# yangjunjie0320/fft-isdf-scratch

Measured on AMD Instinct MI355X. Metric: ISDF build + get_jk k-points/s, diamond gth-dzvp 4x4x4, higher is better.
Workload: dtype f64 (complex128)

## Files before the change

fft-isdf-scratch_amd/csrc/api.hip:

```cpp
#include "../../include/fisdf.h"

#include <algorithm>
#include <cstdlib>
#include <cmath>
#include <cstring>
#include <functional>
#include <map>
#include <mutex>
#include <set>
#include <string>
#include <vector>

#include "common.h"
#include "linalg.h"

namespace fisdf {

static thread_local std::string g_last_error;
static thread_local fisdf_ctx* t_cur_ctx = nullptr;
static std::mutex g_live_mu;
static std::set<const fisdf_ctx*> g_live;
void set_ctx_error(fisdf_ctx* c, const std::string& msg);
void set_error(const std::string& msg) {
  g_last_error = msg;
// ... 56 lines not shown
  bool time_reversal = false;
  double omega = 0.0;
  hipStream_t aux[3] = {nullptr, nullptr, nullptr};
  hipEvent_t ev_fork = nullptr, ev_join[3] = {nullptr, nullptr, nullptr};
  unsigned aux_use[3] = {0, 0, 0}, aux_joined[3] = {0, 0, 0};
  hipEvent_t ev_ybuf[4] = {nullptr, nullptr, nullptr, nullptr};
  std::vector<hipEvent_t> ev_q;
  std::vector<hipEvent_t> ev_free;
  int pipe_mode = -1;
  int pipe_depth = 0;
  int last_fit_lanes = 0, last_fit_pipe = 0;
  struct FitRec {
    int v[12] = {0, 0, 0, 0, 0, 0, 0, 0, 0, 0, 0, 0};
  };
  std::vector<FitRec> fit_report;
  std::vector<hipEvent_t> ev_ready;
  std::vector<char> ready_marked;
  std::vector<const cplx*> y_piece;
  bool y_real_store = false;
  std::vector<char> y_real_slot;
  std::vector<long> y_slices;
  std::map<std::vector<long>, PlaneRef*> plane_cache;
  int* f_piv = nullptr;
  int* f_rank_dev = nullptr;
  std::vector<int> f_rank;
  hipStream_t side = nullptr;
  int factor_hi = 0, side_hi = -1;
  std::vector<hipStream_t> pad;
  void* pad_buf = nullptr;
  hipEvent_t ev_x4 = nullptr, ev_fac = nullptr, ev_chol = nullptr;
  hipEvent_t ev_fac_early = nullptr;
  int f_early = 0;
  bool f_fac_unjoined = false;
  bool f_pending = false;
  bool x4_marked = false;
  int* f_rank_pinned = nullptr;
  void* f_scratch = nullptr;
  size_t f_scratch_size = 0;
  int* stage_pinned = nullptr;
  int* sel_pinned = nullptr;
  size_t sel_cap = 0;
  size_t stage_cap = 0;
  hipEvent_t ev_stage = nullptr;
  unsigned long long* maximag = nullptr;
  unsigned long long* trmon = nullptr;
  unsigned long long* tr_pinned = nullptr;
  hipEvent_t ev_tr = nullptr;
  bool timing = false;
  struct Ev { int stage; hipEvent_t a, b; int span; };
  std::vector<Ev> events;
  unsigned long long* spans = nullptr;
  int span_used = 0;
  static constexpr int kSpanCap = 16384;
  std::string last_error;
  struct Build {
    bool valid = false;
    int nk = 0, nip = 0, nao = 0, ng0 = 0, nfit = 0, used_pivoted = 0, min_norm = 0;
    int time_reversal = 0;
    double tr_deviation = 0.0;
    int kmesh[3] = {0, 0, 0}, mesh[3] = {0, 0, 0};
    double a[9] = {0};
    std::vector<int> perm, fit_qs, partner, ranks;
    std::vector<double> wt;
    void *X = nullptr, *x4 = nullptr, *Wq = nullptr, *Ws = nullptr;
    int shard_rank = 0, shard_size = 1, row0 = 0, row1 = 0;
    void* W0 = nullptr;
    bool sharded = false;
    bool y_streamed = false;
    fisdf_comm comm{};
  } bld;
  hipStream_t comm_stream = nullptr;
  hipEvent_t ev_comm = nullptr;
  fisdf_alloc_fn alloc_fn = nullptr;
  fisdf_free_fn free_fn = nullptr;
  void* alloc_user = nullptr;
  std::map<int, std::pair<void*, size_t>> owned;
  std::vector<void*> lent;
  int* ys_dev = nullptr;
  int* ys_err_pinned = nullptr;
  hipEvent_t ev_yerr = nullptr;
  hipEvent_t ev_ysfork = nullptr;
  hipEvent_t ev_ys2[2] = {nullptr, nullptr};
  DevBuf ws_ypiv, ws_ystream;
  struct YStream {
    bool armed = false, enqueued = false;
    bool stale = false;
    int aux = 2;
    const cplx* x0 = nullptr;
    const cplx* f = nullptr;
    int ng0 = 0, nao = 0, nip = 0, rows = 128;
    long m = 0, fks = 0;
    int kmesh[3] = {0, 0, 0};
    std::vector<int> qs;
    cplx* yT = nullptr;
    unsigned long long rmask = 0;
  } ys;
};

namespace fisdf {
void set_ctx_error(fisdf_ctx* c, const std::string& msg) { c->last_error = msg; }
}

namespace {

static int devbuf_get(fisdf_ctx::DevBuf& w, size_t bytes, void** out) {
  bytes = std::max<size_t>(bytes, 256);
  if (bytes > w.n) {
    if (w.p) {
      FISDF_HIP(hipDeviceSynchronize());
      FISDF_HIP(hipFree(w.p));
    }
    w.p = nullptr;
    w.n = 0;
    FISDF_HIP(hipMalloc(&w.p, bytes));
    w.n = bytes;
  }
  *out = w.p;
  return 0;
}

int arena_get(fisdf_ctx* c, size_t bytes, void** out) {
  bytes = std::max<size_t>(bytes, 256);
  if (bytes > c->arena_size) {
    FISDF_HIP(hipStreamSynchronize(c->stream));
    if (c->arena) FISDF_HIP(hipFree(c->arena));
    c->arena = nullptr;
    c->arena_size = 0;
    size_t sz = bytes + bytes / 8;
    if (hipMalloc(&c->arena, sz) != hipSuccess) {
      (void)hipGetLastError();
      c->arena = nullptr;
      FISDF_HIP(hipMalloc(&c->arena, bytes));
      sz = bytes;
    }
    c->arena_size = sz;
  }
  *out = c->arena;
  return 0;
}

struct Carver {
  size_t off = 0;
  size_t take(size_t bytes) {
    size_t o = off;
    off += (bytes + 255) / 256 * 256;
    return o;
  }
};

int upload_bytes(fisdf_ctx* c, const void* h, size_t bytes, void* d) {
  if (bytes == 0) return 0;
  if (!c->ev_stage) FISDF_HIP(hipEventCreateWithFlags(&c->ev_stage, hipEventDisableTiming));
  FISDF_HIP(hipEventSynchronize(c->ev_stage));
  if (bytes > c->stage_cap) {
    if (c->stage_pinned) FISDF_HIP(hipHostFree(c->stage_pinned));
    c->stage_pinned = nullptr;
    c->stage_cap = 0;
    FISDF_HIP(hipHostMalloc((void**)&c->stage_pinned, bytes, hipHostMallocDefault));
    c->stage_cap = bytes;
  }
  std::memcpy(c->stage_pinned, h, bytes);
  FISDF_HIP(hipMemcpyAsync(d, c->stage_pinned, bytes, hipMemcpyHostToDevice, c->stream));
  FISDF_HIP(hipEventRecord(c->ev_stage, c->stream));
  return 0;
}

// ... 415 lines not shown
}


int pick_ksplit(int M, int N, int K) {
  long tiles = (long)((M + 63) / 64) * ((N + 63) / 64);
  int ks = 1;
  while (tiles * ks < 1024 && K / (ks * 2) >= 512) ks *= 2;
  return ks;
}

constexpr int kLaneWppMinQ = 12;
bool lane_wpp_wanted(int nq) {
  static const int lane_wpp_env = [] {
    const char* e = getenv("FISDF_LANE_WPP");
    return e ? atoi(e) : -1;
  }();
  return lane_wpp_env < 0 ? nq >= kLaneWppMinQ : lane_wpp_env != 0;
}

int wpp_ksplit(int nip) {
  const char* e = getenv("FISDF_WPP_KSPLIT");
  const int v = e ? atoi(e) : 4;
  return (nip >= 256 && v > 1) ? std::min(v, 16) : 1;
}

}

extern "C" {

int fisdf_abi_version(void) { return FISDF_ABI_VERSION; }

const char* fisdf_last_error(const fisdf_ctx* c) {
  return c ? c->last_error.c_str() : g_last_error.c_str();
}

int fisdf_create(int device, void* stream, fisdf_ctx** out) {
  t_cur_ctx = nullptr;
  FISDF_CHECK(out != nullptr, "out is null");
  int ndev = 0;
  FISDF_HIP(hipGetDeviceCount(&ndev));
  FISDF_CHECK(device >= 0 && device < ndev, "device id out of range (no GPU visible?)");
  FISDF_HIP(hipSetDevice(device));
  fisdf_ctx* c = new fisdf_ctx();
  c->device = device;
  c->stream = (hipStream_t)stream;
  c->own_stream = false;
  FISDF_HIP(hipMalloc(&c->maximag, 4 * sizeof(unsigned long long)));
  FISDF_HIP(hipMemsetAsync(c->maximag, 0, 4 * sizeof(unsigned long long), c->stream));
  {
    std::lock_guard<std::mutex> lk(g_live_mu);
    g_live.insert(c);
  }
  *out = c;
  return 0;
}

int fisdf_destroy(fisdf_ctx* c) {
  if (!c) return 0;
  {
    std::lock_guard<std::mutex> lk(g_live_mu);
    g_live.erase(c);
  }
  if (t_cur_ctx == c) t_cur_ctx = nullptr;
  FISDF_HIP(hipSetDevice(c->device));
  FISDF_HIP(hipStreamSynchronize(c->stream));
  c->lent.clear();
  for (auto& kv : c->owned)
    if (kv.second.first) (void)hipFree(kv.second.first);
  c->owned.clear();
  for (auto& e : c->events) { (void)hipEventDestroy(e.a); (void)hipEventDestroy(e.b); }
  for (auto& kv : c->phase_cache) (void)hipFree(kv.second);
  for (auto& kv : c->asym_cache) {
    (void)hipFree(kv.second.idx);
    if (kv.second.f) (void)hipFree(kv.second.f);
  }
  for (auto& kv : c->wt_cache) (void)hipFree(kv.second);
  if (c->f_pending) (void)hipEventSynchronize(c->ev_fac);
  free_factors(c);
  if (c->f_scratch) (void)hipFree(c->f_scratch);
  if (c->f_ring) (void)hipFree(c->f_ring);
  for (int l = 0; l < 3; ++l)
    if (c->aux[l]) (void)hipStreamSynchronize(c->aux[l]);
  if (c->ys_dev) (void)hipFree(c->ys_dev);
  if (c->ys_err_pinned) (void)hipHostFree(c->ys_err_pinned);
  if (c->ev_yerr) (void)hipEventDestroy(c->ev_yerr);
  if (c->ev_ysfork) (void)hipEventDestroy(c->ev_ysfork);
  for (hipEvent_t e : c->ev_ys2)
    if (e) (void)hipEventDestroy(e);
  for (auto* w : {&c->ws_main, &c->ws_side_a, &c->ws_side_b, &c->ws_x4, &c->ws_ypiv, &c->ws_ystream})
    if (w->p) (void)hipFree(w->p);
  for (hipStream_t p : c->pad) (void)hipStreamDestroy(p);
  if (c->pad_buf) (void)hipFree(c->pad_buf);
  if (c->side) {
    (void)hipStreamSynchronize(c->side);
    (void)hipStreamDestroy(c->side);
    (void)hipEventDestroy(c->ev_x4);
    (void)hipEventDestroy(c->ev_fac);
    (void)hipEventDestroy(c->ev_fac_early);
    (void)hipEventDestroy(c->ev_chol);
  }
  if (c->ev_fork) {
    (void)hipEventDestroy(c->ev_fork);
    for (int l = 0; l < 3; ++l) {
      if (c->aux[l]) {
        (void)hipStreamSynchronize(c->aux[l]);
        (void)hipStreamDestroy(c->aux[l]);
        c->aux[l] = nullptr;
      }
      (void)hipEventDestroy(c->ev_join[l]);
    }
    for (int l = 0; l < 4; ++l) (void)hipEventDestroy(c->ev_ybuf[l]);
  }
  for (hipEvent_t e : c->ev_q) (void)hipEventDestroy(e);
  for (hipEvent_t e : c->ev_free) (void)hipEventDestroy(e);
  for (hipEvent_t e : c->ev_ready) (void)hipEventDestroy(e);
  if (c->comm_stream) {
    (void)hipStreamSynchronize(c->comm_stream);
    (void)hipStreamDestroy(c->comm_stream);
    (void)hipEventDestroy(c->ev_comm);
  }
  for (auto& kv : c->plane_cache) (void)hipFree(kv.second);
  if (c->arena) (void)hipFree(c->arena);
  if (c->ev_stage) (void)hipEventSynchronize(c->ev_stage), (void)hipEventDestroy(c->ev_stage);
  if (c->stage_pinned) (void)hipHostFree(c->stage_pinned);
  if (c->sel_pinned) (void)hipHostFree(c->sel_pinned);
  if (c->maximag) (void)hipFree(c->maximag);
  if (c->ev_tr) (void)hipEventSynchronize(c->ev_tr), (void)hipEventDestroy(c->ev_tr);
  if (c->trmon) (void)hipFree(c->trmon);
  if (c->tr_pinned) (void)hipHostFree(c->tr_pinned);
  if (c->spans) (void)hipFree(c->spans);
  if (c->own_stream) (void)hipStreamDestroy(c->stream);
  delete c;
  return 0;
}

int fisdf_sync(fisdf_ctx* c) {
  FISDF_TRY(device_guard(c));
  FISDF_HIP(hipStreamSynchronize(c->stream));
  return 0;
}

int fisdf_malloc(fisdf_ctx* c, size_t bytes, void** p) {
  FISDF_TRY(device_guard(c));
  FISDF_HIP(hipMalloc(p, std::max<size_t>(bytes, 1)));
  return 0;
}

int fisdf_free(fisdf_ctx* c, void* p) {
  FISDF_TRY(device_guard(c));
  FISDF_HIP(hipStreamSynchronize(c->stream));
  FISDF_HIP(hipFree(p));
  return 0;
}

int fisdf_memcpy_htod(fisdf_ctx* c, void* d, const void* h, size_t bytes) {
  FISDF_TRY(device_guard(c));
  FISDF_HIP(hipMemcpyAsync(d, h, bytes, hipMemcpyHostToDevice, c->stream));
  FISDF_HIP(hipStreamSynchronize(c->stream));
  return 0;
}

int fisdf_memcpy_dtoh(fisdf_ctx* c, void* h, const void* d, size_t bytes) {
  FISDF_TRY(device_guard(c));
  FISDF_HIP(hipMemcpyAsync(h, d, bytes, hipMemcpyDeviceToHost, c->stream));
  FISDF_HIP(hipStreamSynchronize(c->stream));
  return 0;
// ... 359 lines not shown
  return 0;
}

int fisdf_trsm_merged_ex(fisdf_ctx* c, const void* Lp, long sL, int r, void* X, long ld, long sX,
                         int ncol, int batch, int lower_rhs, int use_work, long work_elems,
                         int* h_rows, int rows_cap) {
  FISDF_TRY(device_guard(c));
  FISDF_CHECK(r >= 1 && ncol >= 1 && batch >= 1 && ld >= ncol && work_elems >= 0,
              "trsm_merged_ex: bad sizes");
  const int nblk = trsm_merged_blocks(r);
  FISDF_CHECK(!h_rows || rows_cap >= nblk, "trsm_merged_ex: h_rows too short");
  const long rr = (long)r * r;
  Carver cv;
  size_t oQ = cv.take(sizeof(cplx) * (size_t)batch * rr);
  size_t oK = cv.take(sizeof(cplx) * (size_t)std::max(1L, work_elems));
  void* base;
  FISDF_TRY(arena_get(c, cv.off, &base));
  cplx* Q = (cplx*)((char*)base + oQ);
  cplx* work = use_work ? (cplx*)((char*)base + oK) : nullptr;
  if (h_rows)
    for (int b = 0; b < nblk; ++b) {
      TrsmRow row;
      trsm_merged_row(r, ncol, batch, lower_rhs != 0, use_work != 0, work_elems, b, &row);
      const int v[6] = {row.b0, row.m, row.b1, row.nc, row.ks, row.sub};
      std::memcpy(h_rows + 6 * b, v, sizeof(v));
    }
  FISDF_TRY(build_trsm_q(c->stream, (const cplx*)Lp, r, sL, Q, batch, GEMM_FULL));
  const int rc = trsm_merged_batched(c->stream, Q, rr, r, (cplx*)X, ld, sX, ncol, batch,
                                     lower_rhs != 0, work, use_work ? work_elems : 0);
  FISDF_HIP(hipStreamSynchronize(c->stream));
  return rc;
}

int fisdf_scatter_w(fisdf_ctx* c, const void* Wpp, int ldw, long sW, int rmax, const int* d_piv,
                    const int* d_rank, void* W, int nip, int batch) {
  FISDF_TRY(device_guard(c));
  FISDF_CHECK(nip >= 1 && rmax >= 0 && rmax <= nip && ldw >= rmax && batch >= 0,
              "scatter_w: bad sizes");
  FISDF_TRY(scatter_w(c->stream, (const cplx*)Wpp, ldw, sW, rmax, d_piv, d_rank, (cplx*)W, nip,
                      batch));
  FISDF_HIP(hipStreamSynchronize(c->stream));
  return 0;
}

int fisdf_conj_transpose(fisdf_ctx* c, const void* A, int n, long sA, void* B, int batch) {
  FISDF_TRY(device_guard(c));
  FISDF_CHECK(n >= 1 && batch >= 0 && A != B, "conj_transpose: bad arguments");
  FISDF_TRY(conj_transpose(c->stream, (const cplx*)A, n, sA, (cplx*)B, batch));
  FISDF_HIP(hipStreamSynchronize(c->stream));
  return 0;
}

int fisdf_factor_plan(int n, int ncol, int batch, long work_elems, int* h_pchol_path,
                      int* h_pchol_nb, int* h_nblk, int* h_s0, int* h_rows, int rows_cap,
                      long* h_split_work_elems, int* h_sel_rpt, int* h_sel_nb) {
  t_cur_ctx = nullptr;
  FISDF_CHECK(n >= 1 && ncol >= 1 && batch >= 1, "factor_plan: bad sizes");
  const int nblk = trsm_merged_blocks(n);
  FISDF_CHECK(!h_rows || rows_cap >= nblk, "factor_plan: h_rows too short");
  if (h_pchol_path) *h_pchol_path = pchol_path(n);
  if (h_pchol_nb) *h_pchol_nb = PCHOL_NB;
  if (h_nblk) *h_nblk = nblk;
  TrsmRow row;
  trsm_merged_row(n, ncol, batch, false, false, 0, 0, &row);
  if (h_s0) *h_s0 = row.m;
  if (h_rows)
    for (int b = 0; b < nblk; ++b) {
      TrsmRow full, low;
      trsm_merged_row(n, ncol, batch, false, work_elems >= 0, work_elems, b, &full);
      trsm_merged_row(n, ncol, batch, true, work_elems >= 0, work_elems, b, &low);
      const int v[8] = {full.b0, full.m, full.b1, full.ks, full.sub, low.nc, low.ks, low.sub};
      std::memcpy(h_rows + 8 * b, v, sizeof(v));
    }
  if (h_split_work_elems) *h_split_work_elems = trsm_split_work_elems(n, batch);
  int rpt = 0, nb = 0;
  pchol_real_variant(n, &rpt, &nb);
  if (h_sel_rpt) *h_sel_rpt = rpt;
  if (h_sel_nb) *h_sel_nb = nb;
  return 0;
}

static int ensure_side(fisdf_ctx* c);

static int ystream_enqueue(fisdf_ctx* c, const int* piv) {
  fisdf_ctx::YStream& Y = c->ys;
  FISDF_TRY(ensure_side(c));
  FISDF_TRY(ensure_aux(c));
  const int nq = (int)Y.qs.size();
  const size_t yw = y_fused_workspace(Y.kmesh, Y.nip, Y.nao, (int)Y.m);
  FISDF_CHECK(yw > 0 && nq > 0, "streamed y: the fused kernel does not apply");
  void* wb = nullptr;
  FISDF_TRY(devbuf_get(c->ws_ystream, yw, &wb));
  const int ia = [] {
    const char* e = getenv("FISDF_Y_STREAM_AUX");
    const int v = e ? atoi(e) : 2;
    return (v >= 0 && v <= 2) ? v : 2;
  }();
  c->ys.aux = ia;
  hipStream_t ys = c->aux[ia];
  aux_fork(c, ia);
  FISDF_HIP(hipStreamWaitEvent(ys, c->ev_ysfork, 0));
  const char* e2 = getenv("FISDF_Y_STREAM_2S");
  const int i2 = (e2 && e2[0] == '0') ? -1 : (ia == 0 ? 1 : 0);
  if (i2 >= 0 && !c->ev_ys2[0]) {
    FISDF_HIP(hipEventCreateWithFlags(&c->ev_ys2[0], hipEventDisableTiming));
    FISDF_HIP(hipEventCreateWithFlags(&c->ev_ys2[1], hipEventDisableTiming));
  }
  bool handled = false;
  {
    StageTimer tm(c, FISDF_ST_Y, ys);
    FISDF_TRY(y_fused_stream(ys, Y.x0, Y.ng0, Y.nao, piv, c->ys_dev, c->ys_dev + 1, Y.nip, Y.rows,
                             Y.f, Y.fks, (int)Y.m, Y.kmesh, Y.qs.data(), nq, Y.yT,
                             (long)Y.nip * Y.m, Y.m, 0, (cplx*)wb, yw, Y.rmask, &handled,
                             i2 >= 0 ? c->aux[i2] : nullptr, c->ev_ys2[0], c->ev_ys2[1]));
  }
  if (i2 >= 0) {
    aux_fork(c, i2);
    c->aux_joined[i2] = c->aux_use[i2];
  }
  FISDF_CHECK(handled, "streamed y: nothing enqueued");
  Y.enqueued = true;
  return 0;
}

static bool ystream_valid(fisdf_ctx* c, int nip, const int* qs, int nq) {
  const fisdf_ctx::YStream& Y = c->ys;
  return Y.enqueued && !Y.stale && nip == Y.nip && (int)Y.qs.size() == nq &&
         std::equal(Y.qs.begin(), Y.qs.end(), qs);
}

static int ystream_join(fisdf_ctx* c) {
  const int ia = c->ys.aux;
  if (!c->ys.enqueued || c->aux_joined[ia] == c->aux_use[ia]) return 0;
  FISDF_TRY(aux_join(c, ia));
  FISDF_HIP(hipMemcpyAsync(c->ys_err_pinned, c->ys_dev + 1, sizeof(int), hipMemcpyDeviceToHost,
                           c->stream));
  FISDF_HIP(hipEventRecord(c->ev_yerr, c->stream));
  return 0;
}

static int ystream_check(fisdf_ctx* c) {
  FISDF_HIP(hipEventSynchronize(c->ev_yerr));
  FISDF_CHECK(*c->ys_err_pinned == 0, "streamed y: the selection's progress never arrived");
  return 0;
}

static int ystream_arm(fisdf_ctx* c, const void* x0, int ng0, const void* f, long fks, long m,
                       int nao, int nip_max, const int kmesh[3], const int* qs, int nq, void* yT,
                       unsigned long long rmask, bool* armed) {
  *armed = false;
  FISDF_TRY(ystream_join(c));
  c->ys = fisdf_ctx::YStream();
  if (nip_max <= 0 || m <= 0 || nq <= 0 || !y_fused_applies(kmesh, nao)) return 0;
  FISDF_CHECK(x0 && f && yT && qs, "y_stream_arm: null argument");
  if (!c->ys_dev) {
    FISDF_HIP(hipMalloc((void**)&c->ys_dev, 4 * sizeof(int)));
    FISDF_HIP(hipHostMalloc((void**)&c->ys_err_pinned, sizeof(int), hipHostMallocDefault));
    FISDF_HIP(hipEventCreateWithFlags(&c->ev_yerr, hipEventDisableTiming));
    FISDF_HIP(hipEventCreateWithFlags(&c->ev_ysfork, hipEventDisableTiming));
  }
  fisdf_ctx::YStream& Y = c->ys;
  Y.x0 = (const cplx*)x0;
  Y.f = (const cplx*)f;
  Y.fks = fks;
  Y.m = m;
  Y.ng0 = ng0;
  Y.nao = nao;
  Y.nip = std::min(nip_max, ng0);
  for (int i = 0; i < 3; ++i) Y.kmesh[i] = kmesh[i];
  Y.qs.assign(qs, qs + nq);
  Y.yT = (cplx*)yT;
  Y.rmask = rmask;
  const int rows_env = [] {
    const char* e = getenv("FISDF_Y_STREAM_ROWS");
    const int v = e ? atoi(e) : 128;
    return (v >= 16 && v % 16 == 0 && v <= 1024) ? v : 128;
  }();
  Y.rows = rows_env;
  Y.armed = true;
  *armed = true;
  return 0;
}

static size_t select_work_bytes(int n) {
  const size_t nn = (size_t)n * n;
  return std::max(sizeof(cplx) * nn, sizeof(double) * (nn + 17 * (size_t)n + 1));
}

static int select_pivots_dev(fisdf_ctx* c, const cplx* X2, double scale, int ng0, int nip_max,
                             double tol, cplx* X4, int* piv, int* rank, cplx* L, double* d,
                             int* flags, double* w, int* h_perm, int* h_rank,
                             const SelOpts* opt = nullptr, int* h_info = nullptr) {
  const size_t nint = 2 + (size_t)nip_max;
  if (c->sel_cap < nint) {
    if (c->sel_pinned) FISDF_HIP(hipHostFree(c->sel_pinned));
    c->sel_pinned = nullptr;
    c->sel_cap = 0;
// ... 330 lines not shown
}

static int build_x4_on(fisdf_ctx* c, hipStream_t st, fisdf_ctx::DevBuf* wsb, const void* Xv,
                       int nip, int nao, const int kmesh[3], const double a[9], void* x4v);

int fisdf_build_x4(fisdf_ctx* c, const void* Xv, int nip, int nao, const int kmesh[3],
                   const double a[9], void* x4v) {
  FISDF_TRY(device_guard(c));
  return build_x4_on(c, c->stream, nullptr, Xv, nip, nao, kmesh, a, x4v);
}

static int build_x4_on(fisdf_ctx* c, hipStream_t st, fisdf_ctx::DevBuf* wsb, const void* Xv,
                       int nip, int nao, const int kmesh[3], const double a[9], void* x4v) {
  FISDF_TRY(kmesh_check(kmesh, "build_x4"));
  FISDF_CHECK(nip >= 1 && nao >= 1, "build_x4: bad sizes");
  StageTimer tm(c, FISDF_ST_X4, st);
  const int nk = kmesh[0] * kmesh[1] * kmesh[2];
  const cplx* phase;
  FISDF_TRY(get_phase(c, kmesh, a, &phase));
  const cplx* X = (const cplx*)Xv;
  const long nn = (long)nip * nip;
  if (nk == 1) {
    FISDF_TRY(zgemm(st, OP_R, OP_T, nip, nip, nao, ONE, X, nao, 0, X, nao, 0, ZERO,
                    (cplx*)x4v, nip, 0, 1, 1, nullptr, EPI_CSQUARE, c->maximag + 0));
    return 0;
  }
  if (x4_dft_enabled() && kmesh_y_reg_applies(kmesh, nn)) {
    const bool half = c->time_reversal;
    const int nks = half ? kmesh_half_count(kmesh) : nk;
    void* base;
    if (wsb)
      FISDF_TRY(devbuf_get(*wsb, sizeof(cplx) * (size_t)nks * nn, &base));
    else
      FISDF_TRY(arena_get(c, sizeof(cplx) * (size_t)nks * nn, &base));
    cplx* X2k = (cplx*)base;
    std::vector<int> runs = {0, nk};
    if (half) FISDF_TRY(kmesh_rep_runs(kmesh, &runs));
    for (size_t r = 0, slot = 0; r < runs.size(); r += 2) {
      const int k0 = runs[r], nb = runs[r + 1] - runs[r];
      FISDF_TRY(zgemm(st, OP_R, OP_T, nip, nip, nao, ONE, X + (long)k0 * nip * nao, nao,
                      (long)nip * nao, X + (long)k0 * nip * nao, nao, (long)nip * nao, ZERO,
                      X2k + (long)slot * nn, nip, nn, nb));
      slot += nb;
    }
    std::vector<int> all(nk);
    for (int q = 0; q < nk; ++q) all[q] = q;
    FISDF_TRY(kmesh_y(st, X2k, nn, kmesh, all.data(), nullptr, nk, nip, (cplx*)x4v, nn, nip,
                      0, half, c->maximag + 0, true));
    return 0;
  }
  FISDF_CHECK(st == c->stream, "build_x4: the dense path runs on the context stream only");
  Carver cv;
  size_t o1 = cv.take(sizeof(cplx) * nk * nn);
  size_t o2 = cv.take(sizeof(cplx) * nk * nn);
  void* base;
  FISDF_TRY(arena_get(c, cv.off, &base));
  cplx* X2k = (cplx*)((char*)base + o1);
  cplx* X2s = (cplx*)((char*)base + o2);
  FISDF_TRY(zgemm(st, OP_R, OP_T, nip, nip, nao, ONE, X, nao, (long)nip * nao, X, nao,
                  (long)nip * nao, ZERO, X2k, nip, nn, nk));
  FISDF_TRY(zgemm(st, OP_N, OP_N, nk, nn, nk, ONE, phase, nk, 0, X2k, nn, 0, ZERO, X2s, nn,
                  0, 1, 1, nullptr, EPI_CSQUARE, c->maximag + 0));
  FISDF_TRY(zgemm(st, OP_C, OP_N, nk, nn, nk, ONE, phase, nk, 0, X2s, nn, 0, ZERO,
                  (cplx*)x4v, nn, 0, 1));
  return 0;
}

int fisdf_build_y_qs(fisdf_ctx* c, const void* fv, long f_kstride, int g0, int nblk, int ngrid,
                     const void* Xv, int nip, int nao, const int kmesh[3], const double a[9],
                     const int* h_qs, int nq, void* yTv) {
  FISDF_TRY(device_guard(c));
  FISDF_CHECK(g0 >= 0 && nblk >= 0 && g0 + nblk <= ngrid, "build_y: block out of range");
  FISDF_TRY(kmesh_check(kmesh, "build_y"));
  StageTimer tm(c, FISDF_ST_Y);
  const int nk = kmesh[0] * kmesh[1] * kmesh[2];
  FISDF_TRY(check_qlist(h_qs, nq, nk, "build_y"));
  FISDF_CHECK(nq > 0, "build_y: empty q-list");
  const cplx* f = (const cplx*)fv;
  const cplx* X = (const cplx*)Xv;
  cplx* yT = (cplx*)yTv;
  constexpr long yblk_bytes = 2048L << 20;
  const bool half = c->time_reversal;
  c->y_real_slot.assign(nq, 0);
#ifdef FISDF_EXP_NOY
  return 0;
#endif
  if (half && nblk > 0) {
    bool done = false;
    const size_t yw = y_fused_workspace(kmesh, nip, nao, nblk);
    unsigned long long rmask = 0;
    if (c->y_real_store && g0 == 0 && nblk == ngrid && nk <= 64)
      for (int i = 0; i < nq; ++i) {
        const int q = h_qs[i];
        const int i2 = q % kmesh[2], i1 = (q / kmesh[2]) % kmesh[1], i0 = q / (kmesh[1] * kmesh[2]);
        if ((2 * i0) % kmesh[0] == 0 && (2 * i1) % kmesh[1] == 0 && (2 * i2) % kmesh[2] == 0)
          rmask |= 1ull << q;
      }
    if (yw) {
      void* wb = nullptr;
      FISDF_TRY(arena_get(c, yw, &wb));
      FISDF_TRY(y_fused(c->stream, X, nip, nao, f, f_kstride, nblk, kmesh, h_qs, nq, yT,
                        (long)nip * ngrid, ngrid, g0, c->maximag + 1, (cplx*)wb, yw, rmask, &done));
    }
    if (done) {
      for (int i = 0; i < nq; ++i) c->y_real_slot[i] = (rmask >> h_qs[i]) & 1ull ? 1 : 0;
      return 0;
    }
  }
  const int nks = half ? kmesh_half_count(kmesh) : nk;
  std::vector<int> runs = {0, nk};
  if (half) FISDF_TRY(kmesh_rep_runs(kmesh, &runs));
  const long per_g = (long)nks * nip * sizeof(cplx);
  int gb = (int)std::max(64L, std::min<long>(nblk, yblk_bytes / std::max(per_g, 1L)));
  gb = std::min(gb, std::max(nblk, 1));
  const int nbuf = gb < nblk ? 2 : 1;
  Carver cv;
  size_t o1[2];
  for (int i = 0; i < nbuf; ++i) o1[i] = cv.take((size_t)per_g * gb);
  size_t oq = cv.take(sizeof(int) * (size_t)nq);
  void* base;
  FISDF_TRY(arena_get(c, cv.off, &base));
  int* dq = (int*)((char*)base + oq);
  FISDF_TRY(upload_ints(c, h_qs, nq, dq));
  hipStream_t sk = c->stream;
  if (nbuf == 2) {
    FISDF_TRY(ensure_aux(c));
    sk = c->aux[0];
    aux_fork(c, 0);
    FISDF_HIP(hipEventRecord(c->ev_fork, c->stream));
    FISDF_HIP(hipStreamWaitEvent(sk, c->ev_fork, 0));
  }
  const int fx_epi = EPI_STREAM;
  int blk = 0;
  for (int s0 = 0; s0 < nblk; s0 += gb, ++blk) {
    const int m = std::min(gb, nblk - s0);
    const long nm = (long)nip * m;
    const int bi = blk % nbuf;
    cplx* FX = (cplx*)((char*)base + o1[bi]);
    if (nbuf == 2 && blk >= 2) FISDF_HIP(hipStreamWaitEvent(c->stream, c->ev_ybuf[2 + bi], 0));
    for (size_t r = 0, slot = 0; r < runs.size(); r += 2) {
      const int k0 = runs[r], nb = runs[r + 1] - runs[r];
      FISDF_TRY(zgemm(c->stream, OP_N, OP_C, nip, m, nao, ONE, X + (long)k0 * nip * nao, nao,
                      (long)nip * nao, f + (long)k0 * f_kstride + (long)s0 * nao, nao, f_kstride,
                      ZERO, FX + (long)slot * nm, m, nm, nb, 1, nullptr, fx_epi));
      slot += nb;
    }
    if (nbuf == 2) {
      FISDF_HIP(hipEventRecord(c->ev_ybuf[bi], c->stream));
      FISDF_HIP(hipStreamWaitEvent(sk, c->ev_ybuf[bi], 0));
    }
    FISDF_TRY(kmesh_y(sk, FX, nm, kmesh, h_qs, dq, nq, m, yT, (long)nip * ngrid, ngrid,
                      (long)g0 + s0, half, c->maximag + 1));
    if (nbuf == 2) FISDF_HIP(hipEventRecord(c->ev_ybuf[2 + bi], sk));
  }
  if (nbuf == 2) FISDF_TRY(aux_join(c, 0));
  return 0;
}

int fisdf_build_y(fisdf_ctx* c, const void* fv, long f_kstride, int g0, int nblk, int ngrid,
                  const void* Xv, int nip, int nao, const int kmesh[3], const double a[9],
                  int q0, int q1, void* yTv) {
  t_cur_ctx = c;
  FISDF_CHECK(kmesh && kmesh[0] >= 1 && kmesh[1] >= 1 && kmesh[2] >= 1, "build_y: bad k-mesh");
  const int nk = kmesh[0] * kmesh[1] * kmesh[2];
  FISDF_CHECK(0 <= q0 && q0 < q1 && q1 <= nk, "build_y: bad q range");
  std::vector<int> qs = q_range(q0, q1);
  return fisdf_build_y_qs(c, fv, f_kstride, g0, nblk, ngrid, Xv, nip, nao, kmesh, a, qs.data(),
                          (int)qs.size(), yTv);
}

int factor_finish(fisdf_ctx* c, hipStream_t s, const int* rank_dev_src, bool need_linv) {
  const int nk = c->f_nk, nip = c->f_nip, nb = c->f_nb, nblk = (nip + nb - 1) / nb;
  const long nn = (long)nip * nip;
  FISDF_HIP(hipMemcpyAsync(c->f_rank_pinned, rank_dev_src, sizeof(int) * nk, hipMemcpyDeviceToHost, s));
  FISDF_HIP(hipMemcpyAsync(c->f_rank_dev, rank_dev_src, sizeof(int) * nk, hipMemcpyDeviceToDevice, s));
  FISDF_HIP(hipEventRecord(c->ev_chol, s));
  const long sLi = (long)nblk * nb * nb;
  auto operators = [&](int z0, int nz) -> int {
    if (nz <= 0) return 0;
    FISDF_TRY(gather_lp(s, c->f_L + z0 * nn, nip, nip, c->f_piv + (long)z0 * nip,
                        c->f_rank_dev + z0, nip, c->f_Lp + z0 * nn, nz));
    if (need_linv)
      FISDF_TRY(trinv_blocks(s, c->f_Lp + z0 * nn, nip, nip, nn, nb, sLi, c->f_Linv + z0 * sLi,
                             nz));
    FISDF_TRY(build_trsm_q(s, c->f_Lp + z0 * nn, nip, nn, c->f_Q + z0 * nn, nz, GEMM_FULL));
// ... 172 lines not shown
  if (cv.off > c->f_scratch_size) {
    if (c->f_scratch) FISDF_HIP(hipFree(c->f_scratch));
    FISDF_HIP(hipMalloc(&c->f_scratch, cv.off));
    c->f_scratch_size = cv.off;
  }
  char* b = (char*)c->f_scratch;
  c->f_qs.assign(h_qs, h_qs + nq);
  c->f_real.assign(nq, 0);
  for (int i = 0; kmesh && i < nq; ++i) c->f_real[i] = self_conjugate(kmesh, h_qs[i]) ? 1 : 0;
  c->f_nk = nk;
  c->f_nip = nip;
  c->f_tol = tol_rel;
  c->f_used_pivoted = false;
  if (!c->x4_marked) FISDF_HIP(hipEventRecord(c->ev_x4, c->stream));
  c->x4_marked = false;
  FISDF_HIP(hipStreamWaitEvent(c->side, c->ev_x4, 0));
  StageTimer tm(c, FISDF_ST_FACTOR, c->side);
  hipStream_t s = c->side;
  const bool pivoted = c->force_pivoted == 1 || (c->force_pivoted < 0 && pivoted_fit_forced()) ||
                       c->fit_mode == FISDF_FIT_SVD;
  for (int i = 0; i < nq; ++i) {
    c->f_qr_pinned[i] = h_qs[i];
    c->f_qr_pinned[nq + i] = c->f_real[i];
  }
  FISDF_HIP(hipMemcpyAsync(c->f_qr_dev, c->f_qr_pinned, sizeof(int) * 2 * nq, hipMemcpyHostToDevice, s));
  FISDF_TRY(stage_x4(s, (const cplx*)x4all, c->f_qr_dev, nq, nn, c->f_x4s, pivoted ? nullptr : c->f_L));
  if (pivoted) {
    FISDF_TRY(factor_pivoted(c, s));
    c->f_check_fail = false;
  } else {
    FISDF_TRY(chol_unpivoted(s, c->f_L, nip, nk, tol_rel, c->f_piv, (int*)(b + oU),
                             (int*)(b + oFl), (cplx*)(b + oWk)));
    FISDF_HIP(hipMemcpyAsync(c->f_fail_pinned, b + oFl, sizeof(int) * nk, hipMemcpyDeviceToHost, s));
    FISDF_TRY(factor_finish(c, s, (const int*)(b + oU), false));
    c->f_check_fail = true;
  }
  FISDF_HIP(hipEventRecord(c->ev_fac, s));
  c->f_pending = true;
  return 0;
}

int fisdf_set_pivoted_fit(fisdf_ctx* c, int mode) {
  FISDF_TRY(ctx_guard(c));
  FISDF_CHECK(c != nullptr && mode >= -1 && mode <= 1, "set_pivoted_fit: bad mode");
  c->force_pivoted = mode;
  return 0;
}

int fisdf_set_half_grid(fisdf_ctx* c, int mode) {
  FISDF_TRY(ctx_guard(c));
  FISDF_CHECK(c != nullptr && mode >= -1 && mode <= 1, "set_half_grid: mode must be -1, 0 or 1");
  c->half_grid = mode;
  return 0;
}

int fisdf_set_fit_mode(fisdf_ctx* c, int mode) {
  FISDF_TRY(ctx_guard(c));
  FISDF_CHECK(c != nullptr && mode >= FISDF_FIT_LSTSQ && mode <= FISDF_FIT_BASIC,
              "set_fit_mode: mode must be FISDF_FIT_LSTSQ, FISDF_FIT_SVD or FISDF_FIT_BASIC");
  c->fit_mode = mode;
  return 0;
}

int fisdf_min_norm_info(fisdf_ctx* c, int* h_nslots) {
  FISDF_TRY(ctx_guard(c));
  FISDF_CHECK(c != nullptr, "null context");
  int n = 0;
  for (char v : c->f_cod) n += v ? 1 : 0;
  if (h_nslots) *h_nslots = n;
  return 0;
}

int fisdf_set_omega(fisdf_ctx* c, double omega) {
  FISDF_TRY(ctx_guard(c));
  FISDF_CHECK(c != nullptr && std::isfinite(omega), "set_omega: omega must be finite");
  c->omega = omega;
  return 0;
}

int fisdf_set_time_reversal(fisdf_ctx* c, int on) {
  FISDF_TRY(ctx_guard(c));
  FISDF_CHECK(c != nullptr && (on == 0 || on == 1), "set_time_reversal: on must be 0 or 1");
  c->time_reversal = on == 1;
  return 0;
}

int fisdf_set_fit_lanes(fisdf_ctx* c, int lanes) {
  FISDF_TRY(ctx_guard(c));
  FISDF_CHECK(c != nullptr && lanes >= 0 && lanes <= 4, "set_fit_lanes: lanes must be 0..4");
  c->lanes = lanes;
  return 0;
}

int fisdf_set_fit_pipe(fisdf_ctx* c, int mode, int depth) {
  FISDF_TRY(ctx_guard(c));
  FISDF_CHECK(c != nullptr && mode >= -1 && mode <= 1 && depth >= 0 && depth <= 64,
              "set_fit_pipe: mode must be -1..1, depth 0..64");
  c->pipe_mode = mode;
  c->pipe_depth = depth;
  return 0;
}

}

namespace {
int grow_events(std::vector<hipEvent_t>& v, int n) {
  while ((int)v.size() < n) {
    hipEvent_t e;
    FISDF_HIP(hipEventCreateWithFlags(&e, hipEventDisableTiming));
    v.push_back(e);
  }
  return 0;
}

int mark_y_ready_on(fisdf_ctx* c, int j, hipStream_t st) {
  FISDF_CHECK(j >= 0 && j < 4096, "mark_y_ready: bad index");
  FISDF_TRY(grow_events(c->ev_ready, j + 1));
  if ((int)c->ready_marked.size() <= j) c->ready_marked.resize(j + 1, 0);
  FISDF_HIP(hipEventRecord(c->ev_ready[j], st));
  c->ready_marked[j] = 1;
  return 0;
}

int set_y_slices_on(fisdf_ctx* c, int j, const void* recv, int nparts, const long* h_g0,
                    const long* h_ng, hipStream_t st) {
  FISDF_CHECK(recv != nullptr && nparts >= 1 && nparts <= 4096, "set_y_slices: bad piece");
  std::vector<long> sl;
  for (int p = 0; p < nparts; ++p) {
    FISDF_CHECK(h_g0[p] >= 0 && h_ng[p] >= 0, "set_y_slices: bad slice");
    sl.push_back(h_g0[p]);
    sl.push_back(h_ng[p]);
  }
  bool any = false;
  for (const cplx* pc : c->y_piece) any = any || pc != nullptr;
  FISDF_CHECK(!any || sl == c->y_slices, "set_y_slices: every piece of a call has one layout");
  c->y_slices = sl;
  if ((int)c->y_piece.size() <= j) c->y_piece.resize(j + 1, nullptr);
  c->y_piece[j] = (const cplx*)recv;
  return mark_y_ready_on(c, j, st);
}
}

extern "C" {

int fisdf_mark_y_ready(fisdf_ctx* c, int j) {
  FISDF_TRY(device_guard(c));
  return mark_y_ready_on(c, j, c->stream);
}

int fisdf_set_y_slices(fisdf_ctx* c, int j, const void* recv, int nparts, const long* h_g0,
                       const long* h_ng) {
  FISDF_TRY(device_guard(c));
  return set_y_slices_on(c, j, recv, nparts, h_g0, h_ng, c->stream);
}

int fisdf_fit_info(fisdf_ctx* c, int* h_lanes, int* h_pipe_depth) {
  FISDF_TRY(ctx_guard(c));
  FISDF_CHECK(c != nullptr, "null context");
  if (h_lanes) *h_lanes = c->last_fit_lanes;
  if (h_pipe_depth) *h_pipe_depth = c->last_fit_pipe;
  return 0;
}

int fisdf_fit_report(fisdf_ctx* c, int j, int info[12]) {
  FISDF_TRY(ctx_guard(c));
  FISDF_CHECK(c != nullptr && info != nullptr, "fit_report: null argument");
// ... 1516 lines not shown
  if (h_runs || h_nruns) {
    std::vector<int> runs;
    FISDF_TRY(kmesh_rep_runs(kmesh, &runs));
    const int nr = (int)runs.size() / 2;
    FISDF_CHECK(!h_runs || runs_cap >= nr, "kmesh_plan: h_runs too short");
    if (h_nruns) *h_nruns = nr;
    if (h_runs) std::memcpy(h_runs, runs.data(), sizeof(int) * runs.size());
  }
  YFusedPlan yp;
  y_fused_plan(kmesh, nao, &yp);
  if (h_fused) {
    h_fused[0] = yp.applies ? 1 : 0;
    h_fused[1] = yp.nA;
    h_fused[2] = yp.nB;
    h_fused[3] = yp.nkc;
  }
  if (h_slots)
    for (int i = 0; i < 48; ++i) h_slots[i] = i < yp.nA ? yp.kA[i] : (i - yp.nA < yp.nB ? yp.kB[i - yp.nA] : -1);
  if (h_fused_bytes) {
    h_fused_bytes[0] = (long)yp.lds;
    h_fused_bytes[1] = (long)y_fused_workspace(kmesh, nip, nao, m);
  }
  return 0;
}

static int kmesh_test_scratch(fisdf_ctx* c, size_t extra, const int* h_qs, int nq, char** work,
                              unsigned long long** mon, int** dq) {
  Carver cv;
  const size_t oW = cv.take(extra), oM = cv.take(sizeof(unsigned long long)),
               oQ = cv.take(sizeof(int) * (size_t)std::max(nq, 1));
  void* base;
  FISDF_TRY(arena_get(c, cv.off, &base));
  *work = (char*)base + oW;
  *mon = (unsigned long long*)((char*)base + oM);
  *dq = (int*)((char*)base + oQ);
  FISDF_HIP(hipMemsetAsync(*mon, 0, sizeof(unsigned long long), c->stream));
  FISDF_TRY(upload_ints(c, h_qs, nq, *dq));
  return 0;
}

static int kmesh_test_monitor(fisdf_ctx* c, const unsigned long long* mon, double* h_mon) {
  unsigned long long bits = 0;
  FISDF_HIP(hipMemcpyAsync(&bits, mon, sizeof(bits), hipMemcpyDeviceToHost, c->stream));
  FISDF_HIP(hipStreamSynchronize(c->stream));
  if (h_mon) std::memcpy(h_mon, &bits, sizeof(double));
  return 0;
}

int fisdf_kmesh_y_ex(fisdf_ctx* c, const void* FX, long ncol, const int kmesh[3], const int* h_qs,
                     int nq, int m, void* yT, long qs, long Is, long goff, int half, int conj_out,
                     double* h_mon, int* h_route) {
  FISDF_TRY(device_guard(c));
  if (h_route) *h_route = -1;
  FISDF_CHECK(FX && yT && kmesh && ncol >= 0 && m >= 1 && qs >= 0 && Is >= 0 && goff >= 0,
              "kmesh_y_ex: bad arguments");
  FISDF_TRY(kmesh_check(kmesh, "kmesh_y_ex"));
  FISDF_TRY(check_qlist(h_qs, nq, kmesh[0] * kmesh[1] * kmesh[2], "kmesh_y_ex"));
  const KmeshPlan kp = kmesh_route(kmesh, ncol);
  FISDF_CHECK(kp.route != KM_REFUSED, "kmesh_y_ex: too many columns");
  FISDF_CHECK(!conj_out || kp.route == KM_REG,
              "kmesh_y_ex: conj_out needs the register kernel's k-mesh");
  char* work;
  unsigned long long* mon;
  int* dq;
  FISDF_TRY(kmesh_test_scratch(c, 0, h_qs, nq, &work, &mon, &dq));
  FISDF_TRY(kmesh_y(c->stream, (const cplx*)FX, ncol, kmesh, h_qs, dq, nq, m, (cplx*)yT, qs, Is,
                    goff, half != 0, mon, conj_out != 0));
  FISDF_TRY(kmesh_test_monitor(c, mon, h_mon));
  if (h_route && ncol > 0) *h_route = kp.route;
  return 0;
}

int fisdf_y_fused_ex(fisdf_ctx* c, const void* X, int nip, int nao, const void* F, long fks, int m,
                     const int kmesh[3], const int* h_qs, int nq, void* yT, long qs, long Is,
                     long goff, unsigned long long rmask, int* h_handled) {
  FISDF_TRY(device_guard(c));
  if (h_handled) *h_handled = 0;
  FISDF_CHECK(X && F && yT && kmesh && nip >= 1 && nao >= 1 && m >= 1 && fks >= 0 && qs >= 0 &&
                  Is >= 0 && goff >= 0,
              "y_fused_ex: bad arguments");
  FISDF_TRY(kmesh_check(kmesh, "y_fused_ex"));
  FISDF_TRY(check_qlist(h_qs, nq, kmesh[0] * kmesh[1] * kmesh[2], "y_fused_ex"));
  if (!y_fused_applies(kmesh, nao)) return 0;
  const size_t yw = y_fused_workspace(kmesh, nip, nao, m);
  FISDF_CHECK(yw > 0, "y_fused_ex: no workspace for a k-mesh the fused kernel takes");
  char* work;
  unsigned long long* mon;
  int* dq;
  FISDF_TRY(kmesh_test_scratch(c, yw, h_qs, nq, &work, &mon, &dq));
  bool done = false;
  FISDF_TRY(y_fused(c->stream, (const cplx*)X, nip, nao, (const cplx*)F, fks, m, kmesh, h_qs, nq,
                    (cplx*)yT, qs, Is, goff, mon, (cplx*)work, yw, rmask, &done));
  FISDF_HIP(hipStreamSynchronize(c->stream));
  if (h_handled) *h_handled = done ? 1 : 0;
  return 0;
}

int fisdf_y_fused_stream_ex(fisdf_ctx* c, const void* x0, int ng0, int nao, const int* h_piv,
                            int nip, int rows, const void* F, long fks, int m, const int kmesh[3],
                            const int* h_qs, int nq, void* yT, long qs, long Is, long goff,
                            unsigned long long rmask, int two_streams, int* h_handled,
                            int* h_err) {
  FISDF_TRY(device_guard(c));
  if (h_handled) *h_handled = 0;
  if (h_err) *h_err = 0;
  FISDF_CHECK(x0 && F && yT && kmesh && h_piv && ng0 >= 1 && nip >= 1 && nao >= 1 && m >= 1 &&
                  fks >= 0 && qs >= 0 && Is >= 0 && goff >= 0,
              "y_fused_stream_ex: bad arguments");
  FISDF_CHECK(rows >= 16 && rows % 16 == 0 && rows <= 64 * 16, "y_fused_stream_ex: bad row block");
  for (int i = 0; i < nip; ++i)
    FISDF_CHECK(h_piv[i] >= 0 && h_piv[i] < ng0, "y_fused_stream_ex: pivot out of range");
  FISDF_TRY(kmesh_check(kmesh, "y_fused_stream_ex"));
  FISDF_TRY(check_qlist(h_qs, nq, kmesh[0] * kmesh[1] * kmesh[2], "y_fused_stream_ex"));
  if (!y_fused_applies(kmesh, nao)) return 0;
  const size_t yw = y_fused_workspace(kmesh, nip, nao, m);
  FISDF_CHECK(yw > 0, "y_fused_stream_ex: no workspace for a k-mesh the fused kernel takes");
  Carver cv;
  const size_t oW = cv.take(yw), oP = cv.take(sizeof(int) * ((size_t)nip + 2));
  void* base;
  FISDF_TRY(arena_get(c, cv.off, &base));
  int* dpiv = (int*)((char*)base + oP);
  std::vector<int> h(h_piv, h_piv + nip);
  h.push_back(kSelDone);
  h.push_back(0);
  FISDF_TRY(upload_ints(c, h.data(), nip + 2, dpiv));
  hipStream_t s2 = nullptr;
  hipEvent_t ea = nullptr, eb = nullptr;
  int rc = 0;
  bool done = false;
  if (two_streams) {
    if (hipStreamCreateWithFlags(&s2, hipStreamNonBlocking) != hipSuccess ||
        hipEventCreateWithFlags(&ea, hipEventDisableTiming) != hipSuccess ||
        hipEventCreateWithFlags(&eb, hipEventDisableTiming) != hipSuccess) {
      (void)hipGetLastError();
      set_error("fisdf: y_fused_stream_ex: could not create the second stream");
      rc = -2;
    }
  }
  if (rc == 0)
    rc = y_fused_stream(c->stream, (const cplx*)x0, ng0, nao, dpiv, dpiv + nip, dpiv + nip + 1, nip,
                        rows, (const cplx*)F, fks, m, kmesh, h_qs, nq, (cplx*)yT, qs, Is, goff,
                        (cplx*)((char*)base + oW), yw, rmask, &done, s2, ea, eb);
  int err = 0;
  if (s2) (void)hipStreamSynchronize(s2);
  if (rc == 0 && hipMemcpyAsync(&err, dpiv + nip + 1, sizeof(int), hipMemcpyDeviceToHost,
                                c->stream) != hipSuccess) {
    (void)hipGetLastError();
    set_error("fisdf: y_fused_stream_ex: reading the error flag failed");
    rc = -2;
  }
  (void)hipStreamSynchronize(c->stream);
  if (ea) (void)hipEventDestroy(ea);
  if (eb) (void)hipEventDestroy(eb);
  if (s2) (void)hipStreamDestroy(s2);
  if (rc != 0) return rc;
  if (h_handled) *h_handled = done ? 1 : 0;
  if (h_err) *h_err = err;
  return 0;
}

int fisdf_k_wsrho_ex(fisdf_ctx* c, void* B, long ncol, const int kmesh[3], const double a[9],
                     const void* Ws, long ws_Rstride, int use_reg, double* h_mon,
                     int* h_handled) {
  FISDF_TRY(device_guard(c));
  if (h_handled) *h_handled = 0;
  FISDF_CHECK(B && Ws && kmesh && a && ncol >= 1 && ncol < (1L << 31) && ws_Rstride >= ncol,
              "k_wsrho_ex: bad arguments");
  FISDF_TRY(kmesh_check(kmesh, "k_wsrho_ex"));
  const int nk = kmesh[0] * kmesh[1] * kmesh[2];
  const cplx* phase;
  FISDF_TRY(get_phase(c, kmesh, a, &phase));
  char* work;
  unsigned long long* mon;
  int* dq;
  FISDF_TRY(kmesh_test_scratch(c, sizeof(cplx) * (size_t)nk * ncol, nullptr, 0, &work, &mon, &dq));
  bool reg = false;
  FISDF_TRY(k_wsrho_pair(c, kmesh, phase, (cplx*)B, (cplx*)work, ncol, (const double*)Ws,
                         ws_Rstride, use_reg != 0, mon, &reg));
  FISDF_TRY(kmesh_test_monitor(c, mon, h_mon));
  if (h_handled) *h_handled = reg ? 1 : 0;
  return 0;
}

int fisdf_bloch_dft_ex(fisdf_ctx* c, const void* F, long ncol, const int kmesh[3], void* chi,
                       int* h_route) {
  FISDF_TRY(device_guard(c));
  if (h_route) *h_route = -1;
  FISDF_CHECK(F && chi && kmesh && ncol >= 0, "bloch_dft_ex: bad arguments");
  int route = -1;
  FISDF_TRY(bloch_dft(c->stream, (const double*)F, ncol, kmesh, (cplx*)chi, &route));
  FISDF_HIP(hipStreamSynchronize(c->stream));
  if (h_route && ncol > 0) *h_route = route;
  return 0;
}

int fisdf_bloch_band_ex(fisdf_ctx* c, const void* F, long ncol, int nT, const void* ph, int nkb,
                        void* chi) {
  FISDF_TRY(device_guard(c));
  FISDF_CHECK(F && ph && chi, "bloch_band_ex: bad arguments");
  FISDF_TRY(bloch_band(c->stream, (const double*)F, ncol, nT, (const cplx*)ph, nkb, (cplx*)chi));
  FISDF_HIP(hipStreamSynchronize(c->stream));
  return 0;
}

}

namespace {

enum BuildRole { BR_X = 0, BR_X4 = 1, BR_Y = 2, BR_WQ = 3, BR_WS = 4, BR_SEND = 5, BR_WSB = 6,
                 BR_W0 = 7 };

int build_alloc(fisdf_ctx* c, int role, size_t bytes, void** out) {
  bytes = std::max<size_t>(bytes, 256);
  if (c->alloc_fn) {
    void* p = c->alloc_fn(bytes, c->alloc_user);
    FISDF_CHECK(p != nullptr, "build: the caller's allocator returned NULL");
    c->lent.push_back(p);
    *out = p;
    return 0;
  }
  auto& o = c->owned[role];
  if (o.second < bytes) {
    if (o.first) {
      FISDF_HIP(hipStreamSynchronize(c->stream));
      FISDF_HIP(hipFree(o.first));
// ... 657 lines not shown
```

fft-isdf-scratch_amd/csrc/linalg.h:

```cpp
#pragma once
#include "common.h"

#include <vector>

namespace fisdf {

struct CellGeom {
  double a[3][3];
  double b[3][3];
};

int gather_lp(hipStream_t s, const cplx* L, int n, int rmax, const int* piv, const int* rank,
              int rpad, cplx* Lp, int batch);
int trinv_blocks(hipStream_t s, const cplx* Lp, int r, int ldl, long sL, int nb, long sLi,
                 cplx* Linv, int batch);
int build_trsm_q(hipStream_t s, const cplx* Lp, int r, long sL, cplx* Q, int batch, int mode);
int trsm_merged_batched(hipStream_t s, const cplx* Q, long sQ, int r, cplx* X, long ld, long sX,
                        int ncol, int batch, bool lower_rhs = false, cplx* work = nullptr,
                        long work_elems = 0);
int trsm_split_k(int nc, int b1);
long trsm_split_work_elems(int r, int batch);
struct TrsmRow {
  int b0, m, b1;
  int nc;
  int ks;
  int sub;
};
int trsm_merged_blocks(int r);
bool trsm_merged_row(int r, int ncol, int batch, bool lower_rhs, bool have_work, long work_elems,
                     int b, TrsmRow* row);
int set_identity(hipStream_t s, cplx* X, int n, int batch);
int permute_kgm_sel(hipStream_t s, const cplx* x0, const int* h_k, const double* h_sc, int nsel,
                    int ng, int nao, cplx* out);
int tr_check(hipStream_t s, const cplx* a, long ks, long rows, int nao, long rstride,
             const int kmesh[3], unsigned long long* mon);
void kmesh_reps(const int kmesh[3], std::vector<int>* reps, std::vector<char>* self);
int trsm_blocked(hipStream_t s, int lower, const cplx* Lp, long ldl, long sL, int r,
                 const cplx* Linv, long sLi, int nb, cplx* B, long ldb, long sB, cplx* X, long ldx,
                 long sX, int ncol, int batch, int a_real = 0);
int asym_list(hipStream_t s, const double* w, const int mesh[3], const int m[3], int* idx,
              int* count);
int gather_cols(hipStream_t s, const cplx* A, long ld, int r, const int* idx, int n, cplx* out);
int half_prefix_planes(int n0, int m0);
int half_weight(hipStream_t s, double* w, const double* c, const int mesh[3], const int m[3]);
int asym_half(hipStream_t s, const double* c, const int mesh[3], const int m[3], int* idx,
              double* f, int* count);
int gather_cols_scaled(hipStream_t s, const cplx* A, long ld, int r, const int* idx,
                       const double* f, int n, cplx* out);
int add_imag(hipStream_t s, cplx* G, int ldg, const cplx* H, int ldh, int n);
int zero_imag(hipStream_t s, cplx* a, long n);
int stage_x4(hipStream_t s, const cplx* x4all, const int* qr, int nq, long nn, cplx* x4s, cplx* L);
int min_norm_operator(hipStream_t s, const cplx* L, int n, int rmax, int* piv, int r,
                      cplx* M, long ldm, void* work, int* fail, cplx* q_out = nullptr,
                      cplx* rinv_out = nullptr);
size_t min_norm_work_bytes(int n, int r);
int scatter_w(hipStream_t s, const cplx* Wpp, int ldw, long sW, int rmax, const int* piv,
              const int* rank, cplx* W, int nip, int batch);
int conj_transpose(hipStream_t s, const cplx* A, int n, long sA, cplx* B, int batch);
int coulg_weight(hipStream_t s, const int mesh[3], const CellGeom& g, const double k[3],
                 double scale, int take_sqrt, double* w, double omega = 0.0);
int square_real(hipStream_t s, const cplx* in, cplx* out, long n, unsigned long long* maximag);
int csquare(hipStream_t s, cplx* a, long n, unsigned long long* maximag);
int rho_diag(hipStream_t s, const cplx* T, const cplx* X, int nset, int nk, int nip, int nao,
             double scale, cplx* rho);
int scale_rows(hipStream_t s, const cplx* X, const cplx* v, int nset, int nk, int nip, int i0,
               int nb, int nao, cplx* Xv);
int gather_points(hipStream_t s, const cplx* x0, int nk, int ng0, int nao, const int* perm,
                  int nip, cplx* X);
int square_scale(hipStream_t s, const cplx* in, double sc, cplx* out, long n);
int permute_kgm(hipStream_t s, const cplx* x0, int nq, int ng, int nao, cplx* out);
int pair_product(hipStream_t s, const cplx* A, int n1, const cplx* B, int n2, int nip, cplx* P);
int kmesh_half_count(const int kmesh[3]);
size_t y_fused_workspace(const int kmesh[3], int nip, int nao, int m);
int y_fused(hipStream_t s, const cplx* X, int nip, int nao, const cplx* F, long fks, int m,
            const int kmesh[3], const int* h_qs, int nq, cplx* yT, long qs, long Is, long goff,
            unsigned long long* mon, cplx* work, size_t work_bytes, unsigned long long rmask,
            bool* handled);
bool y_fused_applies(const int kmesh[3], int nao);
int y_fused_stream(hipStream_t s, const cplx* x0, int ng0, int nao, const int* piv,
                   const int* progress, int* err, int nip, int rows, const cplx* F, long fks,
                   int m, const int kmesh[3], const int* h_qs, int nq, cplx* yT, long qs, long Is,
                   long goff, cplx* work, size_t work_bytes, unsigned long long rmask,
                   bool* handled, hipStream_t s2 = nullptr, hipEvent_t ev_a = nullptr,
                   hipEvent_t ev_b = nullptr);
int kmesh_rep_runs(const int kmesh[3], std::vector<int>* runs);
int eval_ao(hipStream_t s, const double* d_coords, int ng, int natm, const double* h_atoms, int nsh,
            const int* h_sh_atom, const int* h_sh_l, const int* h_sh_nprim, const double* h_exps,
            const double* h_coefs, int nT, const int* h_tn, const int kmesh[3], const double a[9],
            double rcut, double* F, void* scratch, size_t scratch_size, cplx* chi, int* h_nao,
            int nkb = 0, const double* h_kband = nullptr);
int kmesh_y(hipStream_t s, const cplx* FX, long ncol, const int kmesh[3], const int* h_qs,
            const int* d_qs, int nq, int m, cplx* yT, long qs, long Is, long goff, bool half,
            unsigned long long* mon, bool conj_out = false);
#define FISDF_KM_REG_MESHES(X)                                                                 \
  X(1, 1, 1) X(1, 1, 2) X(2, 2, 2) X(3, 3, 1) X(3, 3, 3) X(4, 4, 4) X(2, 2, 1) X(1, 2, 2)       \
  X(4, 4, 1) X(2, 2, 4)
enum KmeshRoute { KM_REG = 0, KM_LDS = 1, KM_REFUSED = 2 };
struct KmeshPlan {
  int route;
  int CT;
  size_t lds;
};
KmeshPlan kmesh_route(const int kmesh[3], long ncol);
int kmesh_check(const int kmesh[3], const char* who);
bool kmesh_y_reg_applies(const int kmesh[3], long ncol);
struct YFusedPlan {
  bool applies;
  int nA, nB;
  int kA[16], kB[32];
  size_t lds;
  int nkc;
};
void y_fused_plan(const int kmesh[3], int nao, YFusedPlan* out);
int bloch_dft(hipStream_t s, const double* F, long ncol, const int kmesh[3], cplx* chi,
              int* route = nullptr);
int bloch_band(hipStream_t s, const double* F, long ncol, int nT, const cplx* ph, int nkb,
               cplx* chi);
int k_wsrho_reg(hipStream_t s, cplx* B, long ncol, const int kmesh[3], const double* Ws,
                long ws_Rstride, unsigned long long* mon, bool* handled);

constexpr int kJfftSetChunk = 4;
int rho_grid(hipStream_t s, const cplx* f, long fks, int nk, int ngrid, int nao, const cplx* D,
             int nset, cplx* rho);
bool rho_grid_tiled(int nao);
constexpr long kGramWgs = 1024;
void weighted_gram_split(int nk, int ngrid, int nao, int* chunk, int* nsplit);
long weighted_gram_work_elems(int nk, int ngrid, int nao, int nset);
int weighted_gram(hipStream_t s, const cplx* f, long fks, int nk, int ngrid, int nao,
                  const cplx* v, int nset, int conj_v, double scale, cplx* out, cplx* work,
                  long work_elems);
int conj_inplace(hipStream_t s, cplx* a, long n);

constexpr int kKfftGT = 64;
constexpr int kExxMT = 8;
constexpr int kExxNT = 32;
constexpr long kExxRuns = 128;
constexpr long kKfftWorkBytes = 1L << 29;
constexpr int kKfftMaxNao = 1 << 15, kKfftMaxSets = 1 << 10;
int pair_density(hipStream_t s, const cplx* f1, const cplx* f2, int ngrid, int nao, int m0, int m1,
                 cplx* P);
int pair_density_variant(int ni);
int exx_contract(hipStream_t s, const cplx* Z, const cplx* u, const cplx* f1, const int mesh[3],
                 const double* kd, int m0, int m1, int nao, int nset, double scale, int accumulate,
                 cplx* vk, long vk_set, cplx* work, long work_elems);
int exx_contract_variant(int nao);
void exx_grid_split(int ngrid, int nao, int nset, int* run_len, int* nrun);
long exx_contract_work_elems(int ngrid, int nao, int nset, int mc, int set_chunk);

constexpr int kLrRows = 32;
constexpr int kLrSetChunk = 2;
int pair_density_lr(hipStream_t s, const cplx* f1, int nao, const cplx* psi, int ni, long ld,
                    int ngrid, int m0, int m1, cplx* P);
int exx_contract_lr(hipStream_t s, const cplx* Z, const cplx* u, const cplx* f1, const int mesh[3],
                    const double* kd, int m0, int m1, int nao, int ni, const int* seg, int nset,
                    double scale, int accumulate, cplx* vk, long vk_set, cplx* work,
                    long work_elems);

struct KfftPlan {
  int ok = 0;
  int mc = 0, nchunk = 0;
  int run_len = 0, nrun = 0;
  int pair_tw = 0, exx_sc = 0, exx_nn = 0;
  long row_bytes = 0, part_elems = 0;
  long off_rows = 0, off_psi = 0, off_u = 0, off_w = 0, off_part = 0, bytes = 0;
};
void kfft_plan(int nao, long ngrid, int nset, int rows, bool lowrank, long work_bytes,
               KfftPlan* p);
// ... 18 lines not shown
```

fft-isdf-scratch_amd/csrc/linalg.hip:

```cpp
#include "common.h"
#include "linalg.h"

#include <cmath>

namespace fisdf {

namespace {

__global__ void gather_lp_kernel(const cplx* __restrict__ L, int n, int rmax,
                                 const int* __restrict__ piv, const int* __restrict__ rank,
                                 int rpad, cplx* __restrict__ Lp) {
  const int b = blockIdx.y;
  const int r = rank[b];
  L += (long)b * n * rmax;
  piv += (long)b * rmax;
  Lp += (long)b * rpad * rpad;
  long e = blockIdx.x * (long)blockDim.x + threadIdx.x;
  if (e >= (long)rpad * rpad) return;
  int s = (int)(e / rpad), t = (int)(e % rpad);
  cplx v = cmk(0, 0);
  if (s < r && t < r) {
    if (t <= s) v = L[(long)piv[s] * rmax + t];
  } else if (s == t) {
    v = cmk(1, 0);
  }
  Lp[e] = v;
}

__global__ __launch_bounds__(64) void trinv_blocks_kernel(const cplx* __restrict__ Lp, int r,
                                                          int ldl, long sL, int nb, long sLi,
                                                          cplx* __restrict__ Linv) {
  __shared__ cplx Ls[64][65];
  __shared__ cplx Xs[64][65];
  Lp += blockIdx.y * sL;
  Linv += blockIdx.y * sLi;
  const int blk = blockIdx.x;
  const int b0 = blk * nb;
  const int m = min(nb, r - b0);
  const int j = threadIdx.x;
  for (int i = 0; i < m; ++i)
    if (j < m) Ls[i][j] = Lp[(long)(b0 + i) * ldl + b0 + j];
  __syncthreads();
  if (j < m) {
    for (int i = 0; i < m; ++i) {
      cplx s = cmk(i == j ? 1.0 : 0.0, 0.0);
      for (int t = j; t < i; ++t) s = csub(s, cmul(Ls[i][t], Xs[t][j]));
      cplx d = Ls[i][i];
      double den = d.x * d.x + d.y * d.y;
      Xs[i][j] = i < j ? cmk(0, 0) : cmk((s.x * d.x + s.y * d.y) / den, (s.y * d.x - s.x * d.y) / den);
    }
  }
  __syncthreads();
  cplx* out = Linv + (long)blk * nb * nb;
  for (int i = 0; i < nb; ++i)
    if (j < nb) out[i * nb + j] = (i < m && j < m) ? Xs[i][j] : cmk(i == j ? 1.0 : 0.0, 0.0);
}

__global__ __launch_bounds__(256) void trinv_into_kernel(const cplx* __restrict__ Lp, int r,
                                                         int ldl, long sL, int s0,
                                                         cplx* __restrict__ Q, int ldq, long sQ) {
  __shared__ cplx Ls[64][65];
  __shared__ cplx vec[2][64];
  Lp += blockIdx.y * sL;
  Q += blockIdx.y * sQ;
  const int blk = blockIdx.x;
  const int b0 = blk == 0 ? 0 : s0 + (blk - 1) * 64;
  const int m = blk == 0 ? s0 : min(64, r - b0);
  const int t = threadIdx.x, bi = t >> 4, bj = t & 15, r0 = bi * 4, c0 = bj * 4;
  for (int e = t; e < 64 * 64; e += 256) {
    const int i = e >> 6, j = e & 63;
    Ls[i][j] = (i < m && j <= i) ? Lp[(long)(b0 + i) * ldl + b0 + j] : cmk(0, 0);
  }
  __syncthreads();
  cplx x[4][4];
#pragma unroll
  for (int rr = 0; rr < 4; ++rr)
#pragma unroll
    for (int c = 0; c < 4; ++c) x[rr][c] = cmk(r0 + rr == c0 + c ? 1.0 : 0.0, 0.0);
  for (int kb = 0; 4 * kb < m; ++kb) {
#pragma unroll
    for (int kr = 0; kr < 4; ++kr) {
      const int k = 4 * kb + kr, p = kr & 1;
      if (k >= m) break;
      if (bi == kb) {
        const cplx d = Ls[k][k];
        const double den = d.x * d.x + d.y * d.y;
// ... 325 lines not shown
  for (int t = 0; t < N0; ++t) { double s, c; sincospi(2.0 * t / N0, &s, &c); tw0[t] = cmk(c, s); }
#pragma unroll
  for (int t = 0; t < N1; ++t) { double s, c; sincospi(2.0 * t / N1, &s, &c); tw1[t] = cmk(c, s); }
#pragma unroll
  for (int t = 0; t < N2; ++t) { double s, c; sincospi(2.0 * t / N2, &s, &c); tw2[t] = cmk(c, s); }
  const double sc = 1.0 / sqrt((double)NK);
  double mi = 0.0;
  for (int col = blockIdx.x * blockDim.x + threadIdx.x; col < ncol; col += gridDim.x * blockDim.x) {
    cplx v[NK];
#pragma unroll
    for (int k = 0; k < NK; ++k)
      if (!HALF || kmesh_is_rep(k, N0, N1, N2))
        v[k] = FX[(long)(HALF ? kmesh_rep_slot(k, N0, N1, N2) : k) * ncol + col];
#pragma unroll
    for (int k = 0; k < NK; ++k)
      if (HALF && !kmesh_is_rep(k, N0, N1, N2)) v[k] = cconj(v[kmesh_partner(k, N0, N1, N2)]);
    reg_axis_dft<N0, N1 * N2, NK>(v, tw0);
    reg_axis_dft<N1, N2, NK>(v, tw1);
    reg_axis_dft<N2, 1, NK>(v, tw2);
#pragma unroll
    for (int k = 0; k < NK; ++k) {
      const double re = v[k].x * sc;
      mi = fmax(mi, fabs(v[k].y * sc));
      v[k] = cmk(re * re, 0.0);
    }
    reg_axis_dft<N0, N1 * N2, NK>(v, tw0);
    reg_axis_dft<N1, N2, NK>(v, tw1);
    reg_axis_dft<N2, 1, NK>(v, tw2);
    const unsigned I = (unsigned)col / (unsigned)m, g = (unsigned)col - I * (unsigned)m;
    cplx* out = yT + (long)I * Is + goff + g;
#pragma unroll
    for (int k = 0; k < NK; ++k)
      if ((qmask >> k) & 1ull)
        out[(long)__popcll(qmask & ((1ull << k) - 1ull)) * qs] = cmk(v[k].x * sc, csign * v[k].y * sc);
  }
#pragma unroll
  for (int o = 32; o > 0; o >>= 1) mi = fmax(mi, __shfl_xor(mi, o, 64));
  if ((threadIdx.x & 63) == 0 && mon) atomicMax(mon, (unsigned long long)__double_as_longlong(mi));
}

template <int N0, int N1, int N2>
__global__ __launch_bounds__(64) __attribute__((amdgpu_waves_per_eu(1, 2))) void k_wsrho_reg_kernel(
    cplx* __restrict__ B, long ncol, const double* __restrict__ Ws, long ws_Rstride,
    unsigned long long* __restrict__ mon) {
  constexpr int NK = N0 * N1 * N2;
  cplx tw0[N0], tw1[N1], tw2[N2];
#pragma unroll
  for (int t = 0; t < N0; ++t) { double s, c; sincospi(2.0 * t / N0, &s, &c); tw0[t] = cmk(c, s); }
#pragma unroll
  for (int t = 0; t < N1; ++t) { double s, c; sincospi(2.0 * t / N1, &s, &c); tw1[t] = cmk(c, s); }
#pragma unroll
  for (int t = 0; t < N2; ++t) { double s, c; sincospi(2.0 * t / N2, &s, &c); tw2[t] = cmk(c, s); }
  const double sc = 1.0 / sqrt((double)NK);
  double mi = 0.0;
  for (long col = blockIdx.x * (long)blockDim.x + threadIdx.x; col < ncol;
       col += (long)gridDim.x * blockDim.x) {
    cplx v[NK];
#pragma unroll
    for (int k = 0; k < NK; ++k) v[k] = B[(long)k * ncol + col];
    reg_axis_dft<N0, N1 * N2, NK>(v, tw0);
    reg_axis_dft<N1, N2, NK>(v, tw1);
    reg_axis_dft<N2, 1, NK>(v, tw2);
#pragma unroll
    for (int s = 0; s < NK; ++s) {
      mi = fmax(mi, fabs(v[s].y * sc));
      v[s] = cmk(Ws[(long)s * ws_Rstride + col] * (v[s].x * sc), 0.0);
    }
    reg_axis_dft<N0, N1 * N2, NK>(v, tw0);
    reg_axis_dft<N1, N2, NK>(v, tw1);
    reg_axis_dft<N2, 1, NK>(v, tw2);
#pragma unroll
    for (int k = 0; k < NK; ++k) B[(long)k * ncol + col] = cmk(v[k].x * sc, v[k].y * sc);
  }
#pragma unroll
  for (int o = 32; o > 0; o >>= 1) mi = fmax(mi, __shfl_xor(mi, o, 64));
  if ((threadIdx.x & 63) == 0 && mon) atomicMax(mon, (unsigned long long)__double_as_longlong(mi));
}

constexpr int YF_MAXKS = 7;
struct YfPlan {
  int nA, nB;
  int kA[16];
  int kB[32];
};

template <int N1, int N2>
__host__ __device__ constexpr int yf_inplane_partner(int bc) {
  return ((N1 - bc / N2) % N1) * N2 + (N2 - bc % N2) % N2;
}
template <int N1, int N2>
__host__ __device__ constexpr int yf_inplane_rank(int bc) {
  int r = 0;
  for (int j = 0; j < bc; ++j) r += j <= yf_inplane_partner<N1, N2>(j) ? 1 : 0;
  return r;
}

__device__ __forceinline__ void yf_mfma_chunk(const cplx* __restrict__ XT, int nip, int nao,
                                              const cplx* __restrict__ FT, int m, int sbase,
                                              int nslot, int Ia, bool okI,
                                              int ga, bool okg, int lane, int w,
                                              cplx* __restrict__ buf) {
  const int i16 = lane & 15, kq = lane >> 4;
  const int nkc = (nao + 4 * YF_MAXKS - 1) / (4 * YF_MAXKS);
  cplx a0[YF_MAXKS], b0[YF_MAXKS], a1[YF_MAXKS], b1[YF_MAXKS];
  const int Ic = min(Ia, nip - 1), gc = min(ga, m - 1);
  (void)okI;
  (void)okg;
  auto load = [&](cplx (&a)[YF_MAXKS], cplx (&b)[YF_MAXKS], int s, int c) {
    const long sl = (long)(sbase + s) * nao;
    const cplx* xa = XT + sl * nip + Ic;
    const cplx* fb = FT + sl * m + gc;
#pragma unroll
    for (int kk = 0; kk < YF_MAXKS; ++kk) {
      const int mu = min(c * 4 * YF_MAXKS + kk * 4 + kq, nao - 1);
      a[kk] = xa[(long)mu * nip];
      b[kk] = fb[(long)mu * m];
    }
  };
  f64x4 t1 = {0, 0, 0, 0}, t2 = {0, 0, 0, 0}, t3 = {0, 0, 0, 0};
  auto mma = [&](const cplx (&a)[YF_MAXKS], const cplx (&b)[YF_MAXKS], int s, int c, int cn) {
#pragma unroll
    for (int kk = 0; kk < YF_MAXKS; ++kk) {
      if (c * 4 * YF_MAXKS + kk * 4 >= nao) break;
      const bool ok = c * 4 * YF_MAXKS + kk * 4 + kq < nao;
      const double ar = ok ? a[kk].x : 0.0, ai = ok ? a[kk].y : 0.0, br = b[kk].x, bi = b[kk].y;
      t1 = __builtin_amdgcn_mfma_f64_16x16x4f64(ar, br, t1, 0, 0, 0);
      t2 = __builtin_amdgcn_mfma_f64_16x16x4f64(ai, bi, t2, 0, 0, 0);
      t3 = __builtin_amdgcn_mfma_f64_16x16x4f64(ar + ai, br - bi, t3, 0, 0, 0);
    }
    if (cn == 0) {
#pragma unroll
      for (int r = 0; r < 4; ++r)
        buf[s * 256 + (kq + 4 * r) * 16 + i16] = cmk(t1[r] + t2[r], t3[r] - t1[r] + t2[r]);
      t1 = f64x4{0, 0, 0, 0};
      t2 = f64x4{0, 0, 0, 0};
      t3 = f64x4{0, 0, 0, 0};
    }
  };
  auto next = [&](int s, int c, int& sn, int& cn) {
    sn = s;
    cn = c + 1;
    if (cn == nkc) { sn = s + 4; cn = 0; }
  };
  int s = __builtin_amdgcn_readfirstlane(w), c = 0, sl, cl;
  if (s >= nslot) return;
  auto load_item = [&](cplx (&a)[YF_MAXKS], cplx (&b)[YF_MAXKS], int si, int ci) {
    load(a, b, min(si, nslot - 1), si < nslot ? ci : 0);
  };
  auto step = [&](cplx (&al)[YF_MAXKS], cplx (&bl)[YF_MAXKS], const cplx (&am)[YF_MAXKS],
                  const cplx (&bm)[YF_MAXKS]) {
    load_item(al, bl, sl, cl);
    next(sl, cl, sl, cl);
    int sn, cn;
    next(s, c, sn, cn);
    mma(am, bm, s, c, cn);
    s = sn;
    c = cn;
    return s < nslot;
  };
  load(a0, b0, s, 0);
  next(s, c, sl, cl);
  for (;;) {
    if (!step(a1, b1, a0, b0)) break;
    if (!step(a0, b0, a1, b1)) break;
  }
}

__global__ __launch_bounds__(256) void yf_transpose_kernel(const cplx* __restrict__ src,
                                                           long kstride, int nrow, int nao,
                                                           YfPlan plan, cplx* __restrict__ dst) {
  extern __shared__ cplx tile[];
  const int j = blockIdx.y;
  const int k = j < plan.nA ? plan.kA[j] : plan.kB[j - plan.nA];
  const int r0 = blockIdx.x * 64, nr = min(64, nrow - r0), ld = nao + 1;
  const cplx* sp = src + (long)k * kstride + (long)r0 * nao;
  for (int e = threadIdx.x; e < nr * nao; e += 256) {
    const int r = e / nao, mu = e - r * nao;
    tile[r * ld + mu] = sp[e];
  }
  __syncthreads();
  cplx* dp = dst + (long)j * nao * nrow + r0;
  for (int e = threadIdx.x; e < nao * 64; e += 256) {
    const int mu = e >> 6, r = e & 63;
    if (r < nr) dp[(long)mu * nrow + r] = tile[r * ld + mu];
  }
}

constexpr long kXtSpinCap = 3000000;
__global__ __launch_bounds__(256) void yf_xt_stream_kernel(const cplx* __restrict__ x0,
                                                           long kstride, int ng0, int nao,
                                                           const int* __restrict__ piv,
                                                           const int* __restrict__ progress,
                                                           int lo, int hi, int nip, YfPlan plan,
                                                           cplx* __restrict__ XT,
                                                           int* __restrict__ err) {
  extern __shared__ cplx tile[];
  __shared__ int s_p[64];
  if (threadIdx.x == 0) {
    long spins = 0;
    while (__hip_atomic_load(progress, __ATOMIC_RELAXED, __HIP_MEMORY_SCOPE_AGENT) < hi) {
      __builtin_amdgcn_s_sleep(127);
      if (++spins > kXtSpinCap) {
        atomicExch(err, 1);
        break;
      }
    }
  }
  __syncthreads();
  const int j = blockIdx.y;
  const int k = j < plan.nA ? plan.kA[j] : plan.kB[j - plan.nA];
  const int r0 = lo + blockIdx.x * 64, nr = min(64, hi - r0), ld = nao + 1;
  if (threadIdx.x < 64) {
    int p = 0;
    if ((int)threadIdx.x < nr)
      p = __hip_atomic_load(&piv[r0 + threadIdx.x], __ATOMIC_RELAXED, __HIP_MEMORY_SCOPE_AGENT);
    s_p[threadIdx.x] = min(max(p, 0), ng0 - 1);
  }
  __syncthreads();
  const cplx* sp = x0 + (long)k * kstride;
  for (int e = threadIdx.x; e < nr * nao; e += 256) {
    const int r = e / nao, mu = e - r * nao;
    tile[r * ld + mu] = sp[(long)s_p[r] * nao + mu];
  }
  __syncthreads();
  cplx* dp = XT + (long)j * nao * nip + r0;
  for (int e = threadIdx.x; e < nao * 64; e += 256) {
    const int mu = e >> 6, r = e & 63;
    if (r < nr) dp[(long)mu * nip + r] = tile[r * ld + mu];
  }
}

template <int N0, int N1, int N2>
__global__ __launch_bounds__(256) __attribute__((amdgpu_waves_per_eu(2, 2))) void y_fused_kernel(
    const cplx* __restrict__ XT, int nip, int nao, const cplx* __restrict__ FT, int m,
    int nIt, int nGt, YfPlan plan, unsigned long long qmask, unsigned long long rmask,
    cplx* __restrict__ yT, long qs, long Is, long goff, int mode, int gpair, int it0) {
  constexpr int P = N1 * N2, NK = N0 * P;
  constexpr int R = yf_inplane_rank<N1, N2>(P);
  constexpr int NC = (N0 - 1) / 2;
  constexpr int NR = (N0 % 2 == 0 && N0 > 1) ? 2 : 1;
  static_assert(N0 <= 4 && NC <= 1, "y_fused: k-mesh axis 0 must be <= 4");
  extern __shared__ cplx buf[];
  const int tid = threadIdx.x, lane = tid & 63, w = tid >> 6;
  const int xcd = blockIdx.x & 7, j = blockIdx.x >> 3;
  const int grp = j / (nIt * gpair), rem = j - grp * nIt * gpair;
  const int it = rem / gpair, gt = (grp * gpair + rem % gpair) * 8 + xcd;
  if (gt >= nGt) return;
  const int I0 = (it0 + it) * 16, g0 = gt * 16;
  const int Ia = I0 + (lane & 15), ga = g0 + (lane & 15);
  const bool okI = Ia < nip, okg = ga < m;
  cplx tw0[N0], tw1[N1], tw2[N2];
#pragma unroll
  for (int t = 0; t < N0; ++t) { double sn, cs; sincospi(2.0 * t / N0, &sn, &cs); tw0[t] = cmk(cs, sn); }
#pragma unroll
  for (int t = 0; t < N1; ++t) { double sn, cs; sincospi(2.0 * t / N1, &sn, &cs); tw1[t] = cmk(cs, sn); }
#pragma unroll
  for (int t = 0; t < N2; ++t) { double sn, cs; sincospi(2.0 * t / N2, &sn, &cs); tw2[t] = cmk(cs, sn); }
  cplx tc[NC > 0 ? P : 1];
  double tr[NR][P];
  if (!(mode & 1)) yf_mfma_chunk(XT, nip, nao, FT, m, plan.nA, plan.nB, Ia, okI, ga, okg, lane, w, buf);
  __syncthreads();
  if (!(mode & 2)) {
#pragma unroll
    for (int pi = 0; pi < NR; ++pi) {
      cplx u[P];
#pragma unroll
      for (int bc = 0; bc < P; ++bc)
        if (bc <= yf_inplane_partner<N1, N2>(bc))
          u[bc] = (mode & 1) ? cmk(0, 0) : buf[(pi * R + yf_inplane_rank<N1, N2>(bc)) * 256 + tid];
#pragma unroll
      for (int bc = 0; bc < P; ++bc)
        if (bc > yf_inplane_partner<N1, N2>(bc)) u[bc] = cconj(u[yf_inplane_partner<N1, N2>(bc)]);
      reg_axis_dft<N1, N2, P>(u, tw1);
      reg_axis_dft<N2, 1, P>(u, tw2);
#pragma unroll
      for (int bc = 0; bc < P; ++bc) tr[pi][bc] = u[bc].x;
    }
  }
  if constexpr (NC > 0) {
    __syncthreads();
    if (!(mode & 1)) yf_mfma_chunk(XT, nip, nao, FT, m, 0, plan.nA, Ia, okI, ga, okg, lane, w, buf);
    __syncthreads();
    if (mode & 2) return;
#pragma unroll
    for (int bc = 0; bc < P; ++bc) tc[bc] = (mode & 1) ? cmk(0, 0) : buf[bc * 256 + tid];
    reg_axis_dft<N1, N2, P>(tc, tw1);
    reg_axis_dft<N2, 1, P>(tc, tw2);
  }
  if (mode & 2) return;
  const double sc = 1.0 / sqrt((double)NK), sc2 = sc * sc;
  double rr[NR][P];
  cplx rc[NC > 0 ? P : 1];
#pragma unroll
  for (int s = 0; s < P; ++s) {
    double ys[N0];
#pragma unroll
    for (int a2 = 0; a2 < N0; ++a2) {
      double f = tr[0][s];
      if constexpr (NR == 2) f += (a2 & 1) ? -tr[1][s] : tr[1][s];
      if constexpr (NC > 0) {
        const cplx wv = tw0[a2 % N0];
        f += 2.0 * (wv.x * tc[s].x - wv.y * tc[s].y);
      }
      ys[a2] = f * f * sc2;
    }
    double r0 = 0.0, rh = 0.0;
    cplx r1 = cmk(0, 0);
#pragma unroll
    for (int a2 = 0; a2 < N0; ++a2) {
      r0 += ys[a2];
      if constexpr (NR == 2) rh += (a2 & 1) ? -ys[a2] : ys[a2];
      if constexpr (NC > 0) r1 = cadd(r1, cscale(tw0[a2 % N0], ys[a2]));
    }
    rr[0][s] = r0;
    if constexpr (NR == 2) rr[1][s] = rh;
    if constexpr (NC > 0) rc[s] = r1;
  }
  const int I = I0 + (tid >> 4), g = g0 + (tid & 15);
  if (I >= nip || g >= m) return;
  cplx* out = yT + (long)I * Is + goff + g;
  auto put = [&](int q, cplx v) {
    if ((qmask >> q) & 1ull) {
      const long so = (long)__popcll(qmask & ((1ull << q) - 1ull)) * qs;
      if ((rmask >> q) & 1ull) {
        __builtin_nontemporal_store(v.x * sc, (double*)(yT + so) + ((long)I * Is + goff + g));
      } else {
        typedef double dv2 __attribute__((ext_vector_type(2)));
        __builtin_nontemporal_store(dv2{v.x * sc, v.y * sc}, (dv2*)(out + so));
      }
    }
  };
#pragma unroll
  for (int pi = 0; pi < NR; ++pi) {
    cplx u[P];
#pragma unroll
    for (int bc = 0; bc < P; ++bc) u[bc] = cmk(rr[pi][bc], 0.0);
    reg_axis_dft<N1, N2, P>(u, tw1);
    reg_axis_dft<N2, 1, P>(u, tw2);
    const int qa = pi == 0 ? 0 : N0 / 2;
#pragma unroll
    for (int bc = 0; bc < P; ++bc) put(qa * P + bc, u[bc]);
  }
  if constexpr (NC > 0) {
    reg_axis_dft<N1, N2, P>(rc, tw1);
    reg_axis_dft<N2, 1, P>(rc, tw2);
#pragma unroll
    for (int bc = 0; bc < P; ++bc) {
      put(P + bc, rc[bc]);
      put((N0 - 1) * P + yf_inplane_partner<N1, N2>(bc), cconj(rc[bc]));
    }
  }
}

__global__ void pair_product_kernel(const cplx* __restrict__ A, int n1, const cplx* __restrict__ B,
                                    int n2, int nip, cplx* __restrict__ P) {
  long e = blockIdx.x * (long)blockDim.x + threadIdx.x;
  const long tot = (long)nip * n1 * n2;
  if (e >= tot) return;
  const int j = (int)(e % n2);
  const int i = (int)((e / n2) % n1);
  const int I = (int)(e / ((long)n1 * n2));
  P[e] = cmul(cconj(A[(long)I * n1 + i]), B[(long)I * n2 + j]);
}

// ... 654 lines not shown
}

int kmesh_y(hipStream_t s, const cplx* FX, long ncol, const int kmesh[3], const int* h_qs,
            const int* d_qs, int nq, int m, cplx* yT, long qs, long Is, long goff,
            bool half, unsigned long long* mon, bool conj_out) {
  const int nk = kmesh[0] * kmesh[1] * kmesh[2];
  for (int i = 0; i < nq; ++i)
    FISDF_CHECK(h_qs[i] >= 0 && h_qs[i] < nk && (i == 0 || h_qs[i] > h_qs[i - 1]),
                "kmesh_y: q-list must be ascending and inside the k-mesh");
  FISDF_CHECK(kmesh[0] >= 1 && kmesh[1] >= 1 && kmesh[2] >= 1 && kmesh[0] <= KM_MAXN &&
                  kmesh[1] <= KM_MAXN && kmesh[2] <= KM_MAXN,
              "kmesh_y: k-mesh axes must be <= 16");
  FISDF_CHECK(ncol >= 0 && (m >= 1 || ncol == 0) && nq >= 0, "kmesh_y: bad sizes");
  const KmeshPlan kp = kmesh_route(kmesh, ncol);
  if (kp.route == KM_REG) {
    if (ncol == 0) return 0;
    const int nc = (int)ncol;
    unsigned long long qmask = 0;
    for (int i = 0; i < nq; ++i) qmask |= 1ull << h_qs[i];
    const unsigned grid = (unsigned)std::max<long>(1, std::min<long>((ncol + 63) / 64, 32768));
    const double csign = conj_out ? -1.0 : 1.0;
#define FISDF_KM(a, b, c)                                                                      \
  if (kmesh[0] == a && kmesh[1] == b && kmesh[2] == c) {                                       \
    if (half)                                                                                  \
      hipLaunchKernelGGL((kmesh_y_reg_kernel<a, b, c, true>), dim3(grid), dim3(64), 0, s, FX,   \
                         nc, qmask, m, yT, qs, Is, goff, mon, csign);                          \
    else                                                                                       \
      hipLaunchKernelGGL((kmesh_y_reg_kernel<a, b, c, false>), dim3(grid), dim3(64), 0, s, FX,  \
                         nc, qmask, m, yT, qs, Is, goff, mon, csign);                          \
    FISDF_HIP(hipGetLastError());                                                              \
    return 0;                                                                                  \
  }
    FISDF_KM_REG_MESHES(FISDF_KM)
#undef FISDF_KM
  }
  FISDF_CHECK(!conj_out, "kmesh_y: conj_out needs the register kernel's k-mesh");
  const int CT = kp.CT;
  const size_t lds = kp.lds;
  FISDF_CHECK(lds <= 160 * 1024, "kmesh_y: k-mesh too large for the LDS tile");
  FISDF_CHECK(d_qs != nullptr, "kmesh_y: device q-list required for this k-mesh");
  FISDF_CHECK(kp.route == KM_LDS, "kmesh_y: too many columns");
  const long tiles = (ncol + CT - 1) / CT;
  if (tiles == 0) return 0;
  const unsigned grid = (unsigned)std::min<long>(tiles, 4096);
  FISDF_TRY(func_max_lds((const void*)kmesh_y_kernel, 160 * 1024));
  hipLaunchKernelGGL(kmesh_y_kernel, dim3(grid), dim3(256), lds, s, FX, ncol, nk,
                     kmesh[0], kmesh[1], kmesh[2], d_qs, nq, m, yT, qs, Is, goff, CT, half ? 1 : 0, mon);
  FISDF_HIP(hipGetLastError());
  return 0;
}

size_t y_fused_workspace(const int kmesh[3], int nip, int nao, int m) {
  const int n0 = kmesh[0], P = kmesh[1] * kmesh[2];
  if (n0 * P > 64 || n0 > 4 || P > 16 || m <= 0 || nip <= 0 || nao > 128)
    return 0;
  const int nr = (n0 % 2 == 0 && n0 > 1) ? 2 : 1;
  int nslot = n0 >= 3 ? P : 0;
  nslot += nr * P;
  return sizeof(cplx) * (size_t)nslot * nao * ((size_t)nip + m);
}

static int yf_setup(const int kmesh[3], int nao, const int* h_qs, int nq, YfPlan* plan,
                    unsigned long long* qmask, size_t* lds, bool* ok) {
  *ok = false;
  const int n0 = kmesh[0], n1 = kmesh[1], n2 = kmesh[2];
  const int nk = n0 * n1 * n2, P = n1 * n2;
  if (nk > 64 || n0 > 4 || P > 16 || nao > 128) return 0;
  for (int i = 0; i < nq; ++i)
    FISDF_CHECK(h_qs[i] >= 0 && h_qs[i] < nk && (i == 0 || h_qs[i] > h_qs[i - 1]),
                "y_fused: q-list must be ascending and inside the k-mesh");
  *qmask = 0;
  for (int i = 0; i < nq; ++i) *qmask |= 1ull << h_qs[i];
  *plan = YfPlan{};
  if (n0 >= 3)
    for (int bc = 0; bc < P; ++bc) plan->kA[plan->nA++] = P + bc;
  const int nr = (n0 % 2 == 0 && n0 > 1) ? 2 : 1;
  for (int pi = 0; pi < nr; ++pi) {
    const int a = pi == 0 ? 0 : n0 / 2;
    for (int bc = 0; bc < P; ++bc) {
      const int b = bc / n2, c = bc % n2;
      if (bc <= ((n1 - b) % n1) * n2 + (n2 - c) % n2) plan->kB[plan->nB++] = a * P + bc;
    }
  }
  *lds = sizeof(cplx) * 256 * (size_t)std::max(plan->nA, plan->nB);
  *ok = *lds <= 80 * 1024;
  return 0;
}

static int yf_launch(hipStream_t s, const int kmesh[3], const cplx* XT, int nip, int nao,
                     const cplx* FT, int m, int it0, int nIt, const YfPlan& plan,
                     unsigned long long qmask, unsigned long long rmask, cplx* yT, long qs,
                     long Is, long goff, size_t lds, bool* handled) {
  const int n0 = kmesh[0], n1 = kmesh[1], n2 = kmesh[2];
  const int nGt = (m + 15) / 16;
  constexpr int gpair = 4;
  const long grid = (long)nIt * ((nGt + 8 * gpair - 1) / (8 * gpair)) * gpair * 8;
  FISDF_CHECK(grid < (1L << 31), "y_fused: grid too large");
  FISDF_CHECK(it0 >= 0 && nIt >= 1 && (it0 + nIt - 1) * 16 < nip, "y_fused: I-tiles out of range");
  static const int mode = getenv("FISDF_YF_MODE") ? atoi(getenv("FISDF_YF_MODE")) : 0;
#define FISDF_YF(a, b, c)                                                                      \
  if (n0 == a && n1 == b && n2 == c) {                                                         \
    FISDF_TRY(func_max_lds((const void*)y_fused_kernel<a, b, c>, 80 * 1024));                \
    hipLaunchKernelGGL((y_fused_kernel<a, b, c>), dim3((unsigned)grid), dim3(256), lds, s, XT,  \
                       nip, nao, FT, m, nIt, nGt, plan, qmask, rmask & qmask, yT, qs, Is, goff, \
                       mode, gpair, it0);                                                     \
    FISDF_HIP(hipGetLastError());                                                              \
    *handled = true;                                                                           \
    return 0;                                                                                  \
  }
  FISDF_KM_REG_MESHES(FISDF_YF)
#undef FISDF_YF
  return 0;
}

int y_fused(hipStream_t s, const cplx* X, int nip, int nao, const cplx* F, long fks, int m,
            const int kmesh[3], const int* h_qs, int nq, cplx* yT, long qs, long Is, long goff,
            unsigned long long* mon, cplx* work, size_t work_bytes, unsigned long long rmask,
            bool* handled) {
  (void)mon;
  *handled = false;
  if (m <= 0 || nip <= 0) return 0;
  YfPlan plan;
  unsigned long long qmask = 0;
  size_t lds = 0;
  bool ok = false;
  FISDF_TRY(yf_setup(kmesh, nao, h_qs, nq, &plan, &qmask, &lds, &ok));
  if (!ok || kmesh_route(kmesh, 1).route != KM_REG) return 0;
  const int nsl = plan.nA + plan.nB;
  FISDF_CHECK(work && work_bytes >= sizeof(cplx) * (size_t)nsl * nao * ((size_t)nip + m),
              "y_fused: workspace too small");
  cplx* XT = work;
  cplx* FT = work + (size_t)nsl * nao * nip;
  const size_t tl = sizeof(cplx) * 64 * (size_t)(nao + 1);
  FISDF_TRY(func_max_lds((const void*)yf_transpose_kernel, 132 * 1024));
  hipLaunchKernelGGL(yf_transpose_kernel, dim3((nip + 63) / 64, nsl), dim3(256), tl, s, X,
                     (long)nip * nao, nip, nao, plan, XT);
  FISDF_HIP(hipGetLastError());
  hipLaunchKernelGGL(yf_transpose_kernel, dim3((m + 63) / 64, nsl), dim3(256), tl, s, F, fks, m,
                     nao, plan, FT);
  FISDF_HIP(hipGetLastError());
  return yf_launch(s, kmesh, XT, nip, nao, FT, m, 0, (nip + 15) / 16, plan, qmask, rmask, yT, qs,
                   Is, goff, lds, handled);
}

bool y_fused_applies(const int kmesh[3], int nao) {
  YFusedPlan p;
  y_fused_plan(kmesh, nao, &p);
  return p.applies;
}

void y_fused_plan(const int kmesh[3], int nao, YFusedPlan* out) {
  *out = YFusedPlan{};
  if (nao < 1 || kmesh_route(kmesh, 1).route != KM_REG) return;
  YfPlan plan;
  unsigned long long qmask = 0;
  size_t lds = 0;
  bool ok = false;
  const int q0 = 0;
  if (yf_setup(kmesh, nao, &q0, 1, &plan, &qmask, &lds, &ok) != 0 || !ok) return;
  out->applies = true;
  out->nA = plan.nA;
  out->nB = plan.nB;
  for (int i = 0; i < plan.nA; ++i) out->kA[i] = plan.kA[i];
  for (int i = 0; i < plan.nB; ++i) out->kB[i] = plan.kB[i];
  out->lds = lds;
  out->nkc = (nao + 4 * YF_MAXKS - 1) / (4 * YF_MAXKS);
}

int y_fused_stream(hipStream_t s, const cplx* x0, int ng0, int nao, const int* piv,
                   const int* progress, int* err, int nip, int rows, const cplx* F, long fks,
                   int m, const int kmesh[3], const int* h_qs, int nq, cplx* yT, long qs, long Is,
                   long goff, cplx* work, size_t work_bytes, unsigned long long rmask,
                   bool* handled, hipStream_t s2, hipEvent_t ev_a, hipEvent_t ev_b) {
  *handled = false;
  if (m <= 0 || nip <= 0) return 0;
  FISDF_CHECK(rows >= 16 && rows % 16 == 0 && rows <= 64 * 16, "y_fused_stream: bad row block");
  FISDF_CHECK(!s2 || (ev_a && ev_b), "y_fused_stream: a second stream needs two events");
  YfPlan plan;
  unsigned long long qmask = 0;
  size_t lds = 0;
  bool ok = false;
  FISDF_TRY(yf_setup(kmesh, nao, h_qs, nq, &plan, &qmask, &lds, &ok));
  if (!ok) return 0;
  FISDF_CHECK(kmesh_route(kmesh, 1).route == KM_REG, "y_fused_stream: no kernel for this k-mesh");
  const int nsl = plan.nA + plan.nB;
  FISDF_CHECK(work && work_bytes >= sizeof(cplx) * (size_t)nsl * nao * ((size_t)nip + m),
              "y_fused_stream: workspace too small");
  cplx* XT = work;
  cplx* FT = work + (size_t)nsl * nao * nip;
  const size_t tl = sizeof(cplx) * 64 * (size_t)(nao + 1);
  FISDF_TRY(func_max_lds((const void*)yf_transpose_kernel, 132 * 1024));
  FISDF_TRY(func_max_lds((const void*)yf_xt_stream_kernel, 132 * 1024));
  hipLaunchKernelGGL(yf_transpose_kernel, dim3((m + 63) / 64, nsl), dim3(256), tl, s, F, fks, m,
                     nao, plan, FT);
  FISDF_HIP(hipGetLastError());
  if (s2) {
    FISDF_HIP(hipEventRecord(ev_a, s));
    FISDF_HIP(hipStreamWaitEvent(s2, ev_a, 0));
  }
  for (int lo = 0, b = 0; lo < nip; lo += rows, ++b) {
    const int hi = std::min(nip, lo + rows);
    hipStream_t sb = (s2 && (b & 1)) ? s2 : s;
    hipLaunchKernelGGL(yf_xt_stream_kernel, dim3((hi - lo + 63) / 64, nsl), dim3(256), tl, sb, x0,
                       (long)ng0 * nao, ng0, nao, piv, progress, lo, hi, nip, plan, XT, err);
    FISDF_HIP(hipGetLastError());
    bool h = false;
    FISDF_TRY(yf_launch(sb, kmesh, XT, nip, nao, FT, m, lo / 16, (hi - lo + 15) / 16, plan, qmask,
                        rmask, yT, qs, Is, goff, lds, &h));
    FISDF_CHECK(h, "y_fused_stream: no kernel for this k-mesh");
  }
  if (s2) {
    FISDF_HIP(hipEventRecord(ev_b, s2));
    FISDF_HIP(hipStreamWaitEvent(s, ev_b, 0));
  }
  *handled = true;
  return 0;
}

int pair_product(hipStream_t s, const cplx* A, int n1, const cplx* B, int n2, int nip, cplx* P) {
  long n = (long)nip * n1 * n2;
  if (n == 0) return 0;
  hipLaunchKernelGGL(pair_product_kernel, dim3(nblocks(n, 256, 1L << 30)), dim3(256), 0, s, A, n1,
                     B, n2, nip, P);
  FISDF_HIP(hipGetLastError());
  return 0;
}

struct KgmSel {
  int k[64];
  double sc[64];
};
__global__ void permute_kgm_sel_kernel(const cplx* __restrict__ x0, KgmSel sel, int j0, int nchunk,
                                       int nsel, int ng, int nao, cplx* __restrict__ out) {
  long e = blockIdx.x * (long)blockDim.x + threadIdx.x;
  const long tot = (long)nchunk * ng * nao;
  if (e >= tot) return;
  const int m = (int)(e % nao);
  const int g = (int)((e / nao) % ng);
  const int j = (int)(e / ((long)nao * ng));
  out[(long)g * nsel * nao + (long)(j0 + j) * nao + m] =
      cscale(x0[((long)sel.k[j] * ng + g) * nao + m], sel.sc[j]);
}

int permute_kgm_sel(hipStream_t s, const cplx* x0, const int* h_k, const double* h_sc, int nsel,
                    int ng, int nao, cplx* out) {
  FISDF_CHECK(nsel >= 1, "permute_kgm_sel: no k-points");
  for (int j0 = 0; j0 < nsel; j0 += 64) {
    const int nc = std::min(64, nsel - j0);
    KgmSel sel;
    for (int j = 0; j < nc; ++j) {
      sel.k[j] = h_k[j0 + j];
      sel.sc[j] = h_sc[j0 + j];
    }
    const long n = (long)nc * ng * nao;
    hipLaunchKernelGGL(permute_kgm_sel_kernel, dim3(nblocks(n, 256, 1L << 30)), dim3(256), 0, s,
                       x0, sel, j0, nc, nsel, ng, nao, out);
    FISDF_HIP(hipGetLastError());
  }
  return 0;
}

void kmesh_reps(const int kmesh[3], std::vector<int>* reps, std::vector<char>* self) {
  const int nk = kmesh[0] * kmesh[1] * kmesh[2];
  reps->clear();
  self->clear();
  for (int k = 0; k < nk; ++k) {
    const int p = kmesh_partner(k, kmesh[0], kmesh[1], kmesh[2]);
    if (k <= p) {
      reps->push_back(k);
      self->push_back(k == p ? 1 : 0);
    }
  }
}

__global__ void tr_check_kernel(const cplx* __restrict__ a, long ks, long per_k, int nao,
                                long rstride, int n0, int n1, int n2,
                                unsigned long long* __restrict__ mon) {
  const int nk = n0 * n1 * n2;
  double dev = 0.0, mag = 0.0;
  const long tot = (long)nk * per_k;
  for (long e = blockIdx.x * (long)blockDim.x + threadIdx.x; e < tot;
       e += (long)gridDim.x * blockDim.x) {
    const int k = (int)(e / per_k);
    const long i = e - (long)k * per_k;
    const long r = (i / nao) * rstride * nao + i % nao;
    const int p = kmesh_partner(k, n0, n1, n2);
    if (p < k) continue;
    const cplx u = a[k * ks + r];
    const cplx v = p == k ? u : a[p * ks + r];
    dev = fmax(dev, fmax(fabs(v.x - u.x), fabs(v.y + u.y)));
    mag = fmax(mag, fmax(fabs(u.x), fabs(u.y)));
// ... 64 lines not shown
```

fft-isdf-scratch_amd/fisdf/_lib.py:

```python
from __future__ import annotations

import ctypes as C
import os

import numpy as np

_HERE = os.path.dirname(os.path.abspath(__file__))
LIB_PATH = os.path.join(_HERE, "libfisdf%s.so" % (
    "_" + os.environ["FISDF_LIB_VARIANT"] if os.environ.get("FISDF_LIB_VARIANT") else ""))

STAGES = ["select", "x4", "y", "factor", "fft", "trsm", "herk", "small", "get_j", "get_k", "ws",
          "ao"]

_lib = None

_vp = C.c_void_p
_i = C.c_int
_l = C.c_long
_d = C.c_double
_ip = C.POINTER(C.c_int)
_dp = C.POINTER(C.c_double)

_SIGS = {
    "fisdf_abi_version": ([], _i),
    "fisdf_create": ([_i, _vp, C.POINTER(_vp)], _i),
    "fisdf_destroy": ([_vp], _i),
    "fisdf_last_error": ([_vp], C.c_char_p),
    "fisdf_sync": ([_vp], _i),
    "fisdf_malloc": ([_vp, C.c_size_t, C.POINTER(_vp)], _i),
    "fisdf_free": ([_vp, _vp], _i),
    "fisdf_memcpy_htod": ([_vp, _vp, _vp, C.c_size_t], _i),
    "fisdf_memcpy_dtoh": ([_vp, _vp, _vp, C.c_size_t], _i),
    "fisdf_set_timing": ([_vp, _i], _i),
    "fisdf_timings": ([_vp, _dp, _ip], _i),
    "fisdf_max_imag": ([_vp, _dp], _i),
    "fisdf_select_points": ([_vp, _vp, _i, _i, _i, _i, _d, _ip, _ip, _ip], _i),
    "fisdf_select_points_km": ([_vp, _vp, _ip, _i, _i, _i, _d, _ip, _ip, _ip], _i),
    "fisdf_gather_points": ([_vp, _vp, _i, _i, _i, _ip, _i, _vp], _i),
    "fisdf_eval_ao": ([_vp, _vp, _i, _i, _dp, _i, _ip, _ip, _ip, _dp, _dp, _i, _ip, _ip, _dp, _d,
                       _i, _vp], _i),
    "fisdf_eval_ao_band": ([_vp, _vp, _i, _i, _dp, _i, _ip, _ip, _ip, _dp, _dp, _i, _ip, _i, _dp,
                            _dp, _d, _i, _vp], _i),
    "fisdf_get_j_band_rows": ([_vp, _vp, _vp, _vp, _i, _i, _i, _i, _vp, _i, _i, _i, _vp], _i),
    "fisdf_select_gram": ([_vp, _vp, _i, _i, _i, _i, _i, _vp], _i),
    "fisdf_select_pivots": ([_vp, _vp, _i, _i, _i, _d, _ip, _ip, _ip], _i),
    "fisdf_unpack_slices": ([_vp, _vp, _i, _i, C.POINTER(_l), C.POINTER(_l), _l, _vp], _i),
    "fisdf_build_x4": ([_vp, _vp, _i, _i, _ip, _dp, _vp], _i),
    "fisdf_build_y": ([_vp, _vp, _l, _i, _i, _i, _vp, _i, _i, _ip, _dp, _i, _i, _vp], _i),
    "fisdf_factor_x4": ([_vp, _vp, _i, _i, _i, _d, _ip], _i),
    "fisdf_fit_coulomb": ([_vp, _i, _i, _vp, _i, _ip, _ip, _dp, _vp], _i),
    "fisdf_build_ws": ([_vp, _vp, _i, _i, _i, _ip, _dp, _vp], _i),
    "fisdf_build_y_qs": ([_vp, _vp, _l, _i, _i, _i, _vp, _i, _i, _ip, _dp, _ip, _i, _vp], _i),
    "fisdf_factor_x4_qs": ([_vp, _vp, _ip, _i, _i, _d, _ip, _ip], _i),
    "fisdf_factor_x4_async": ([_vp, _vp, _ip, _i, _i, _d, _ip], _i),
    "fisdf_factor_x4_wait": ([_vp, _ip], _i),
    "fisdf_factor_x4_mark": ([_vp], _i),
    "fisdf_set_omega": ([_vp, _d], _i),
    "fisdf_set_pivoted_fit": ([_vp, _i], _i),
    "fisdf_factor_info": ([_vp, _ip], _i),
    "fisdf_set_fit_mode": ([_vp, _i], _i),
    "fisdf_set_half_grid": ([_vp, _i], _i),
    "fisdf_min_norm_operator": ([_vp, _vp, _i, _d, _vp, _vp, _vp, _ip, _ip], _i),
    "fisdf_min_norm_info": ([_vp, _ip], _i),
    "fisdf_set_fit_lanes": ([_vp, _i], _i),
    "fisdf_set_factor_priority": ([_vp, _i], _i),
    "fisdf_set_time_reversal": ([_vp, _i], _i),
    "fisdf_set_fit_pipe": ([_vp, _i, _i], _i),
    "fisdf_fit_info": ([_vp, _ip, _ip], _i),
    "fisdf_fit_report": ([_vp, _i, _ip], _i),
    "fisdf_fit_plan": ([_ip, _ip, _i, _i, _i, _ip], _i),
    "fisdf_mark_y_ready": ([_vp, _i], _i),
    "fisdf_set_y_slices": ([_vp, _i, _vp, _i, C.POINTER(_l), C.POINTER(_l)], _i),
    "fisdf_reserve_workspace": ([_vp, C.c_size_t], _i),
    "fisdf_fit_coulomb_qs": ([_vp, _ip, _i, _vp, _i, _ip, _ip, _dp, _vp], _i),
    "fisdf_build_ws_qs": ([_vp, _vp, _ip, _dp, _i, _i, _ip, _dp, _vp], _i),
    "fisdf_get_j": ([_vp, _vp, _vp, _vp, _i, _i, _i, _i, _vp], _i),
    "fisdf_get_k": ([_vp, _vp, _vp, _vp, _i, _i, _i, _ip, _dp, _vp], _i),
    "fisdf_get_j_rows": ([_vp, _vp, _vp, _vp, _i, _i, _i, _i, _i, _i, _vp], _i),
    "fisdf_get_k_rows": ([_vp, _vp, _vp, _vp, _i, _i, _i, _ip, _dp, _i, _i, _vp], _i),
    "fisdf_get_k_rows_local": ([_vp, _vp, _vp, _vp, _i, _i, _i, _ip, _dp, _i, _i, _vp], _i),
    "fisdf_build_ws_rows": ([_vp, _vp, _ip, _dp, _i, _i, _ip, _dp, _i, _i, _vp], _i),
    "fisdf_build_ws_blocks": ([_vp, _vp, _ip, _dp, _i, _i, _ip, _dp, _i, _ip, _l, _vp], _i),
    "fisdf_get_rho": ([_vp, _vp, _l, _i, _i, _i, _vp, _i, _vp], _i),
    "fisdf_coulomb_potential": ([_vp, _vp, _i, _ip, _dp, _d, _vp], _i),
    "fisdf_weighted_gram": ([_vp, _vp, _l, _i, _i, _i, _vp, _i, _i, _d, _vp], _i),
    "fisdf_get_j_fft": ([_vp, _vp, _l, _ip, _ip, _dp, _i, _vp, _i, _d, _vp, _i, _vp], _i),
    "fisdf_pair_density": ([_vp, _vp, _vp, _i, _i, _i, _i, _vp], _i),
    "fisdf_exx_contract": ([_vp, _vp, _vp, _vp, _ip, _dp, _i, _i, _i, _i, _d, _vp], _i),
    "fisdf_get_k_fft": ([_vp, _vp, _l, _ip, _ip, _dp, _i, _vp, _i, _d, _vp, _dp, _i, _l, _vp], _i),
    "fisdf_kfft_plan": ([_i, _l, _i, _l, _ip, _ip, _ip, _ip, _ip, _ip, C.POINTER(_l),
                         C.POINTER(_l)], _i),
    "fisdf_pair_density_lr": ([_vp, _vp, _i, _vp, _i, _l, _i, _i, _i, _vp], _i),
    "fisdf_exx_contract_lr": ([_vp, _vp, _vp, _vp, _ip, _dp, _i, _i, _i, _i, _ip, _i, _d, _vp], _i),
    "fisdf_get_k_fft_lr": ([_vp, _vp, _l, _ip, _ip, _dp, _i, _vp, _vp, _ip, _i, _i, _d, _vp, _dp,
                            _i, _l, _vp], _i),
    "fisdf_kfft_lr_plan": ([_i, _l, _i, _i, _l, _ip, _ip, _ip, _ip, _ip, _ip, _ip, C.POINTER(_l),
                            C.POINTER(_l)], _i),
    "fisdf_pair34": ([_vp, C.POINTER(_vp), C.POINTER(_vp), _i, _i, _i, _l, _l, _ip, _dp, _i, _i,
                      _vp], _i),
    "fisdf_get_eri_fft": ([_vp, _ip, _dp, _dp, _d, _vp, _i, _vp, _i, C.POINTER(_vp),
                           C.POINTER(_vp), _i, _i, _i, _l, _vp], _i),
    "fisdf_eri_fft_plan": ([_i, _i, _i, _i, _i, _l, _l, _ip, _ip, _ip, _ip, _ip, _ip, _ip,
                            C.POINTER(_l)], _i),
    "fisdf_get_eri": ([_vp, _vp, _i, _i, _ip, _vp, C.POINTER(_vp), _ip, _vp], _i),
    "fisdf_zgemm": ([_vp, _i, _i, _i, _i, _i, _dp, _vp, _l, _l, _vp, _l, _l, _dp, _vp, _l, _l,
                     _i, _i], _i),
    "fisdf_zgemm_mode": ([_vp, _i, _i, _i, _i, _i, _dp, _vp, _l, _l, _vp, _l, _l, _dp, _vp, _l,
                          _l, _i, _i], _i),
    "fisdf_zgemm_ex": ([_vp, _i, _i, _i, _i, _i, _dp, _vp, _l, _l, _vp, _l, _l, _dp, _vp, _l, _l,
                        _i, _i, _i, _i, _vp, _l, _dp], _i),
    "fisdf_herk_ex": ([_vp, _i, _i, _d, _vp, _l, _l, _d, _vp, _l, _l, _i, _i, _i], _i),
    "fisdf_herk": ([_vp, _i, _i, _d, _vp, _l, _vp, _l, _i], _i),
    "fisdf_fft3d": ([_vp, _vp, _vp, _i, _ip], _i),
    "fisdf_fft3d_paired": ([_vp, _vp, _vp, _i, _ip, _dp, _ip, _i], _i),
    "fisdf_fft3d_ex": ([_vp, _vp, _l, _vp, _vp, _l, _i, _ip, _dp, _vp, C.POINTER(_l), C.POINTER(_l),
                        _ip, _i, _ip], _i),
    "fisdf_coulg": ([_vp, _ip, _dp, _dp, _d, _i, _vp], _i),
    "fisdf_pivoted_cholesky": ([_vp, _vp, _i, _i, _i, _d, _ip, _ip], _i),
    "fisdf_cholesky": ([_vp, _vp, _i, _i, _d, _ip], _i),
    "fisdf_tri_inverse": ([_vp, _vp, _i, _i, _vp], _i),
    "fisdf_pivoted_cholesky_ex": ([_vp, _vp, _l, _l, _i, _i, _i, _d, _d, _vp, _vp, _vp, _ip], _i),
    "fisdf_gather_lp": ([_vp, _vp, _i, _i, _vp, _vp, _i, _vp, _i], _i),
    "fisdf_trsm_blocked_ex": ([_vp, _i, _vp, _l, _l, _i, _vp, _l, _l, _vp, _l, _l, _i, _i, _i], _i),
    "fisdf_trsm_merged_ex": ([_vp, _vp, _l, _i, _vp, _l, _l, _i, _i, _i, _i, _l, _ip, _i], _i),
    "fisdf_scatter_w": ([_vp, _vp, _i, _l, _i, _vp, _vp, _vp, _i, _i], _i),
    "fisdf_conj_transpose": ([_vp, _vp, _i, _l, _vp, _i], _i),
    "fisdf_factor_plan": ([_i, _i, _i, _l, _ip, _ip, _ip, _ip, _ip, _i, C.POINTER(_l), _ip, _ip],
                          _i),
    "fisdf_kmesh_plan": ([_ip, _l, _i, _i, _i, C.POINTER(_l), _ip, _ip, _i, _ip, _ip, _ip,
                          C.POINTER(_l)], _i),
    "fisdf_kmesh_y_ex": ([_vp, _vp, _l, _ip, _ip, _i, _i, _vp, _l, _l, _l, _i, _i, _dp, _ip], _i),
    "fisdf_y_fused_ex": ([_vp, _vp, _i, _i, _vp, _l, _i, _ip, _ip, _i, _vp, _l, _l, _l,
                          C.c_ulonglong, _ip], _i),
    "fisdf_y_fused_stream_ex": ([_vp, _vp, _i, _i, _ip, _i, _i, _vp, _l, _i, _ip, _ip, _i, _vp, _l,
                                 _l, _l, C.c_ulonglong, _i, _ip, _ip], _i),
    "fisdf_k_wsrho_ex": ([_vp, _vp, _l, _ip, _dp, _vp, _l, _i, _dp, _ip], _i),
    "fisdf_bloch_dft_ex": ([_vp, _vp, _l, _ip, _vp, _ip], _i),
    "fisdf_bloch_band_ex": ([_vp, _vp, _l, _i, _vp, _i, _vp], _i),
    "fisdf_select_plan": ([_i, _i, _i, _i, _i, _ip, _ip, C.POINTER(_l), _ip, C.POINTER(_l), _ip,
                           _ip], _i),
    "fisdf_select_pivots_ex": ([_vp, _vp, _i, _i, _i, _d, _i, _i, _i, _ip, _ip, _ip, _ip], _i),
    "fisdf_select_gram_ex": ([_vp, _vp, _ip, _i, _i, _i, _i, _i, _i, _vp, _ip], _i),
    "fisdf_select_gram_plan": ([_ip, _i, _i, _i, _i, _i, _i, _ip], _i),
    "fisdf_build_opts_default": ([_vp], None),
    "fisdf_build": ([_vp, _vp, _i, _vp, _i, _ip, _ip, _dp, _vp, _ip], _i),
    "fisdf_build_y_streamed": ([_vp, _ip], _i),
    "fisdf_y_stream_arm": ([_vp, _vp, _i, _vp, _l, _i, _i, _i, _ip, _ip, _i, _vp, _ip], _i),
    "fisdf_y_stream_finish": ([_vp, _i, _ip], _i),
    "fisdf_build_get": ([_vp, _vp], _i),
# ... 144 lines not shown
```

include/fisdf.h:

```cpp
#ifndef FISDF_H
#define FISDF_H

#include <stddef.h>

#ifdef __cplusplus
extern "C" {
#endif

#define FISDF_ABI_VERSION 4

typedef struct fisdf_ctx fisdf_ctx;

enum {
  FISDF_ST_SELECT = 0,
  FISDF_ST_X4 = 1,
  FISDF_ST_Y = 2,
  FISDF_ST_FACTOR = 3,
  FISDF_ST_FFT = 4,
  FISDF_ST_TRSM = 5,
  FISDF_ST_HERK = 6,
  FISDF_ST_SMALL = 7,
  FISDF_ST_J = 8,
  FISDF_ST_K = 9,
  FISDF_ST_WS = 10,
// ... 95 lines not shown

int fisdf_get_x(fisdf_ctx* ctx, void* h_x);
int fisdf_get_w0(fisdf_ctx* ctx, void* h_w0);
int fisdf_get_wq(fisdf_ctx* ctx, void* h_wq);

int fisdf_get_jk(fisdf_ctx* ctx, const void* d_dms, int nset, int with_j, int with_k, void* d_vj,
                 void* d_vk);

typedef void* (*fisdf_alloc_fn)(size_t bytes, void* user);
typedef void (*fisdf_free_fn)(void* d_ptr, void* user);
int fisdf_set_allocator(fisdf_ctx* ctx, fisdf_alloc_fn alloc, fisdf_free_fn release, void* user);

int fisdf_eval_ao(fisdf_ctx* ctx, const void* d_coords, int ng, int natm, const double* h_atoms,
                  int nsh, const int* h_sh_atom, const int* h_sh_l, const int* h_sh_nprim,
                  const double* h_exps, const double* h_coefs, int nT, const int* h_tn,
                  const int kmesh[3], const double a[9], double rcut, int nao, void* d_out);

int fisdf_eval_ao_band(fisdf_ctx* ctx, const void* d_coords, int ng, int natm, const double* h_atoms,
                       int nsh, const int* h_sh_atom, const int* h_sh_l, const int* h_sh_nprim,
                       const double* h_exps, const double* h_coefs, int nT, const int* h_tn,
                       int nkb, const double* h_kpts, const double a[9], double rcut, int nao,
                       void* d_out);

int fisdf_select_points(fisdf_ctx* ctx, const void* d_x0, int nk, int ng0, int nao, int nip_max,
                        double tol, int* h_perm, int* h_npiv, int* h_full_rank);
int fisdf_select_points_km(fisdf_ctx* ctx, const void* d_x0, const int kmesh[3], int ng0, int nao,
                           int nip_max, double tol, int* h_perm, int* h_npiv, int* h_full_rank);

int fisdf_select_gram(fisdf_ctx* ctx, const void* d_x0, int nk, int q0, int q1, int ng0, int nao,
                      void* d_x2);
int fisdf_select_pivots(fisdf_ctx* ctx, const void* d_x2, int nk, int ng0, int nip_max, double tol,
                        int* h_perm, int* h_npiv, int* h_full_rank);

int fisdf_unpack_slices(fisdf_ctx* ctx, const void* d_recv, int nrows, int nparts,
                        const long* h_g0, const long* h_ng, long ngrid, void* d_yT);

int fisdf_gather_points(fisdf_ctx* ctx, const void* d_x0, int nk, int ng0, int nao,
                        const int* h_perm, int nip, void* d_X);

int fisdf_build_x4(fisdf_ctx* ctx, const void* d_X, int nip, int nao, const int kmesh[3],
                   const double a[9], void* d_x4);

int fisdf_build_y(fisdf_ctx* ctx, const void* d_f, long f_kstride, int g0, int nblk, int ngrid,
                  const void* d_X, int nip, int nao, const int kmesh[3], const double a[9],
                  int q0, int q1, void* d_yT);

int fisdf_build_y_qs(fisdf_ctx* ctx, const void* d_f, long f_kstride, int g0, int nblk, int ngrid,
                     const void* d_X, int nip, int nao, const int kmesh[3], const double a[9],
                     const int* h_qs, int nq, void* d_yT);

int fisdf_factor_x4(fisdf_ctx* ctx, const void* d_x4, int q0, int q1, int nip, double tol_rel,
                    int* h_ranks);
int fisdf_factor_x4_qs(fisdf_ctx* ctx, const void* d_x4, const int* h_qs, int nq, int nip,
                       double tol_rel, const int* kmesh, int* h_ranks);
int fisdf_factor_x4_async(fisdf_ctx* ctx, const void* d_x4, const int* h_qs, int nq, int nip,
                          double tol_rel, const int* kmesh);
int fisdf_factor_x4_wait(fisdf_ctx* ctx, int* h_ranks );
int fisdf_factor_x4_mark(fisdf_ctx* ctx);
int fisdf_set_pivoted_fit(fisdf_ctx* ctx, int mode);
int fisdf_factor_info(fisdf_ctx* ctx, int* h_used_pivoted);
#define FISDF_FIT_LSTSQ 0
#define FISDF_FIT_SVD 1
#define FISDF_FIT_BASIC 2
int fisdf_set_fit_mode(fisdf_ctx* ctx, int mode);
int fisdf_set_half_grid(fisdf_ctx* ctx, int mode);
int fisdf_min_norm_info(fisdf_ctx* ctx, int* h_nslots);

int fisdf_fit_coulomb(fisdf_ctx* ctx, int q0, int q1, const void* d_yT, int nip,
                      const int mesh[3], const int kmesh[3], const double a[9], void* d_Wq);
int fisdf_fit_coulomb_qs(fisdf_ctx* ctx, const int* h_qs, int nq, const void* d_yT, int nip,
                         const int mesh[3], const int kmesh[3], const double a[9], void* d_Wq);
int fisdf_set_fit_lanes(fisdf_ctx* ctx, int lanes);
int fisdf_set_factor_priority(fisdf_ctx* ctx, int high);
int fisdf_set_fit_pipe(fisdf_ctx* ctx, int mode, int depth);
int fisdf_fit_info(fisdf_ctx* ctx, int* h_lanes, int* h_pipe_depth);
int fisdf_fit_report(fisdf_ctx* ctx, int j, int info[12]);
int fisdf_fit_plan(const int kmesh[3], const int mesh[3], int q, int nq, int nip, int info[8]);
int fisdf_mark_y_ready(fisdf_ctx* ctx, int j);
int fisdf_set_y_slices(fisdf_ctx* ctx, int j, const void* d_recv, int nparts, const long* h_g0,
                       const long* h_ng);
int fisdf_reserve_workspace(fisdf_ctx* ctx, size_t bytes);
int fisdf_set_omega(fisdf_ctx* ctx, double omega);
int fisdf_set_time_reversal(fisdf_ctx* ctx, int on);

int fisdf_build_ws(fisdf_ctx* ctx, const void* d_Wq, int q0, int q1, int nip,
                   const int kmesh[3], const double a[9], void* d_Ws);
int fisdf_build_ws_qs(fisdf_ctx* ctx, const void* d_Wq, const int* h_qs, const double* h_wt,
                      int nq, int nip, const int kmesh[3], const double a[9], void* d_Ws);

int fisdf_build_ws_rows(fisdf_ctx* ctx, const void* d_Wq, const int* h_qs, const double* h_wt,
                        int nq, int nip, const int kmesh[3], const double a[9], int i0, int i1,
                        void* d_Ws);
int fisdf_build_ws_blocks(fisdf_ctx* ctx, const void* d_Wq, const int* h_qs, const double* h_wt,
                          int nq, int nip, const int kmesh[3], const double a[9], int nblk,
                          const int* h_rows, long chunk, void* d_Wsb);

int fisdf_get_j(fisdf_ctx* ctx, const void* d_X, const void* d_W0, const void* d_dms, int nset,
                int nk, int nip, int nao, void* d_vj);

int fisdf_get_k(fisdf_ctx* ctx, const void* d_X, const void* d_Ws, const void* d_dms, int nset,
                int nip, int nao, const int kmesh[3], const double a[9], void* d_vk);

int fisdf_get_j_rows(fisdf_ctx* ctx, const void* d_X, const void* d_W0, const void* d_dms,
                     int nset, int nk, int nip, int nao, int i0, int i1, void* d_vj);
int fisdf_get_k_rows(fisdf_ctx* ctx, const void* d_X, const void* d_Ws, const void* d_dms,
                     int nset, int nip, int nao, const int kmesh[3], const double a[9], int i0,
                     int i1, void* d_vk);
int fisdf_get_k_rows_local(fisdf_ctx* ctx, const void* d_X, const void* d_Ws_rows,
                           const void* d_dms, int nset, int nip, int nao, const int kmesh[3],
                           const double a[9], int i0, int i1, void* d_vk);
int fisdf_get_j_band_rows(fisdf_ctx* ctx, const void* d_X, const void* d_W0, const void* d_dms,
                          int nset, int nk, int nip, int nao, const void* d_Xb, int nkb, int i0,
                          int i1, void* d_vj);

int fisdf_get_rho(fisdf_ctx* ctx, const void* d_f, long f_kstride, int nk, int ngrid, int nao,
                  const void* d_dms, int nset, void* d_rho);
int fisdf_coulomb_potential(fisdf_ctx* ctx, const void* d_rho, int nset, const int mesh[3],
                            const double a[9], double omega, void* d_v);
int fisdf_weighted_gram(fisdf_ctx* ctx, const void* d_f, long f_kstride, int nk, int ngrid,
                        int nao, const void* d_v, int nset, int conj_v, double scale, void* d_out);
int fisdf_get_j_fft(fisdf_ctx* ctx, const void* d_f, long f_kstride, const int kmesh[3],
                    const int mesh[3], const double a[9], int nao, const void* d_dms, int nset,
                    double omega, const void* d_fband, int nband, void* d_vj);

int fisdf_pair_density(fisdf_ctx* ctx, const void* d_f1, const void* d_f2, int ngrid, int nao,
                       int m0, int m1, void* d_out);
int fisdf_exx_contract(fisdf_ctx* ctx, const void* d_z, const void* d_u, const void* d_f1,
                       const int mesh[3], const double* h_kd , int m0, int m1,
                       int nao, int nset, double scale, void* d_vk_k1);
int fisdf_get_k_fft(fisdf_ctx* ctx, const void* d_f, long f_kstride, const int kmesh[3],
                    const int mesh[3], const double a[9], int nao, const void* d_dms, int nset,
                    double omega, const void* d_fband, const double* h_kband, int nband,
                    long work_bytes, void* d_vk);
int fisdf_kfft_plan(int nao, long ngrid, int nset, long work_bytes, int* h_mc, int* h_nchunk,
                    int* h_run_len, int* h_nrun, int* h_pair_tw, int* h_exx_nn, long* h_row_bytes,
                    long* h_bytes);

int fisdf_pair_density_lr(fisdf_ctx* ctx, const void* d_f1, int nao, const void* d_psi, int ni,
                          long ld_psi, int ngrid, int m0, int m1, void* d_out);
int fisdf_exx_contract_lr(fisdf_ctx* ctx, const void* d_z, const void* d_u, const void* d_f1,
                          const int mesh[3], const double* h_kd , int m0, int m1,
                          int nao, int ni, const int* h_seg , int nset,
                          double scale, void* d_vk_k1);
int fisdf_get_k_fft_lr(fisdf_ctx* ctx, const void* d_f, long f_kstride, const int kmesh[3],
                       const int mesh[3], const double a[9], int nao, const void* d_A,
                       const void* d_B, const int* h_rank , int rmax, int nset,
                       double omega, const void* d_fband, const double* h_kband, int nband,
                       long work_bytes, void* d_vk);
int fisdf_kfft_lr_plan(int nao, long ngrid, int nset, int imax, long work_bytes, int* h_mc,
                       int* h_nchunk, int* h_run_len, int* h_nrun, int* h_pair_tw, int* h_exx_sc,
                       int* h_exx_nn, long* h_row_bytes, long* h_bytes);

int fisdf_pair34(fisdf_ctx* ctx, const void* const* h_d_a3, const void* const* h_d_a4, int npair,
                 int n3, int n4, long ld3, long ld4, const int mesh[3],
                 const double* h_kd , int r0, int r1, void* d_out);
int fisdf_get_eri_fft(fisdf_ctx* ctx, const int mesh[3], const double a[9], const double h_q[3],
                      double omega, const void* d_a1, int n1, const void* d_a2, int n2,
                      const void* const* h_d_a3, const void* const* h_d_a4, int npair, int n3,
                      int n4, long work_bytes, void* d_out );
int fisdf_eri_fft_plan(int n1, int n2, int n3, int n4, int npair, long ngrid, long work_bytes,
                       int* h_mc, int* h_nrow_chunks, int* h_bc, int* h_nb_chunks, int* h_b_once,
                       int* h_tw, int* h_ksplit, long* h_bytes);

int fisdf_get_eri(fisdf_ctx* ctx, const void* d_X, int nip, int nao, const int kidx[4],
                  const void* d_Wq, const void* const* h_dC, const int nmo[4], void* d_out);

// ... 90 lines not shown
```

Before: 832.6.

## Use real-valued MFMA for self-conjugate k-points in fused Y kernel

For time-reversal-invariant (self-conjugate) k-points in the fused Y contraction, the transposed X and F slices are checked at runtime for negligible imaginary parts. Slots that pass are computed with a single real f64 MFMA product instead of the three-product complex scheme. This adds real-valued copies in the workspace, stats-reduction and flag kernels, and per-slot ordering logic. The aim is fewer FLOPs in the Y build, at the cost of extra transpose work, a larger workspace and extra small kernel launches. It is on by default and can be disabled through an environment variable or a new API call.

```diff
diff --git a/fft-isdf-scratch_amd/csrc/api.hip b/fft-isdf-scratch_amd/csrc/api.hip
--- a/fft-isdf-scratch_amd/csrc/api.hip
+++ b/fft-isdf-scratch_amd/csrc/api.hip
@@ -162,6 +162,9 @@
   hipEvent_t ev_ysfork = nullptr;
   hipEvent_t ev_ys2[2] = {nullptr, nullptr};
   DevBuf ws_ypiv, ws_ystream;
+  int y_realk = -1;
+  unsigned long long* yrk_dev = nullptr;
+  int yrk_last = -1, yrk_slots = 0;
   struct YStream {
     bool armed = false, enqueued = false;
     bool stale = false;
@@ -743,6 +746,7 @@
   for (int l = 0; l < 3; ++l)
     if (c->aux[l]) (void)hipStreamSynchronize(c->aux[l]);
   if (c->ys_dev) (void)hipFree(c->ys_dev);
+  if (c->yrk_dev) (void)hipFree(c->yrk_dev);
   if (c->ys_err_pinned) (void)hipHostFree(c->ys_err_pinned);
   if (c->ev_yerr) (void)hipEventDestroy(c->ev_yerr);
   if (c->ev_ysfork) (void)hipEventDestroy(c->ev_ysfork);
@@ -1268,15 +1272,40 @@
 
 static int ensure_side(fisdf_ctx* c);
 
+constexpr size_t kYrkWords = 130;
+static int yrk_get(fisdf_ctx* c, int set, const int kmesh[3], int nao, YfRealK* rk) {
+  *rk = YfRealK();
+  YFusedPlan yp;
+  y_fused_plan(kmesh, nao, &yp);
+  c->yrk_slots = yp.applies ? yp.nA + yp.nB : 0;
+  c->yrk_last = -1;
+  static const bool env_on = [] {
+    const char* e = getenv("FISDF_Y_REALK");
+    return !(e && e[0] == '0');
+  }();
+  if (!(c->y_realk < 0 ? env_on : c->y_realk == 1) || !yp.applies) return 0;
+  if (!c->yrk_dev) {
+    FISDF_HIP(hipMalloc((void**)&c->yrk_dev, 2 * kYrkWords * sizeof(unsigned long long)));
+    FISDF_HIP(hipMemset(c->yrk_dev, 0, 2 * kYrkWords * sizeof(unsigned long long)));
+  }
+  rk->stats = c->yrk_dev + set * kYrkWords;
+  rk->flags = (unsigned*)(rk->stats + 128);
+  c->yrk_last = set;
+  return 0;
+}
+
 static int ystream_enqueue(fisdf_ctx* c, const int* piv) {
   fisdf_ctx::YStream& Y = c->ys;
   FISDF_TRY(ensure_side(c));
   FISDF_TRY(ensure_aux(c));
   const int nq = (int)Y.qs.size();
-  const size_t yw = y_fused_workspace(Y.kmesh, Y.nip, Y.nao, (int)Y.m);
+  const size_t yw = y_fused_workspace(Y.kmesh, Y.nip, Y.nao, (int)Y.m) +
+                    y_fused_real_workspace(Y.kmesh, Y.nip, Y.nao, (int)Y.m);
   FISDF_CHECK(yw > 0 && nq > 0, "streamed y: the fused kernel does not apply");
   void* wb = nullptr;
   FISDF_TRY(devbuf_get(c->ws_ystream, yw, &wb));
+  YfRealK rk;
+  FISDF_TRY(yrk_get(c, 1, Y.kmesh, Y.nao, &rk));
   const int ia = [] {
     const char* e = getenv("FISDF_Y_STREAM_AUX");
     const int v = e ? atoi(e) : 2;
@@ -1298,7 +1327,7 @@
     FISDF_TRY(y_fused_stream(ys, Y.x0, Y.ng0, Y.nao, piv, c->ys_dev, c->ys_dev + 1, Y.nip, Y.rows,
                              Y.f, Y.fks, (int)Y.m, Y.kmesh, Y.qs.data(), nq, Y.yT,
                              (long)Y.nip * Y.m, Y.m, 0, (cplx*)wb, yw, Y.rmask, &handled,
-                             i2 >= 0 ? c->aux[i2] : nullptr, c->ev_ys2[0], c->ev_ys2[1]));
+                             i2 >= 0 ? c->aux[i2] : nullptr, c->ev_ys2[0], c->ev_ys2[1], rk));
   }
   if (i2 >= 0) {
     aux_fork(c, i2);
@@ -1795,12 +1824,15 @@
   constexpr long yblk_bytes = 2048L << 20;
   const bool half = c->time_reversal;
   c->y_real_slot.assign(nq, 0);
+  c->yrk_last = -1;
+  c->yrk_slots = 0;
 #ifdef FISDF_EXP_NOY
   return 0;
 #endif
   if (half && nblk > 0) {
     bool done = false;
-    const size_t yw = y_fused_workspace(kmesh, nip, nao, nblk);
+    const size_t yw0 = y_fused_workspace(kmesh, nip, nao, nblk);
+    const size_t yw = yw0 ? yw0 + y_fused_real_workspace(kmesh, nip, nao, nblk) : 0;
     unsigned long long rmask = 0;
     if (c->y_real_store && g0 == 0 && nblk == ngrid && nk <= 64)
       for (int i = 0; i < nq; ++i) {
@@ -1812,8 +1844,11 @@
     if (yw) {
       void* wb = nullptr;
       FISDF_TRY(arena_get(c, yw, &wb));
+      YfRealK rk;
+      FISDF_TRY(yrk_get(c, 0, kmesh, nao, &rk));
       FISDF_TRY(y_fused(c->stream, X, nip, nao, f, f_kstride, nblk, kmesh, h_qs, nq, yT,
-                        (long)nip * ngrid, ngrid, g0, c->maximag + 1, (cplx*)wb, yw, rmask, &done));
+                        (long)nip * ngrid, ngrid, g0, c->maximag + 1, (cplx*)wb, yw, rmask, &done,
+                        rk));
     }
     if (done) {
       for (int i = 0; i < nq; ++i) c->y_real_slot[i] = (rmask >> h_qs[i]) & 1ull ? 1 : 0;
@@ -2152,6 +2187,27 @@
   FISDF_TRY(ctx_guard(c));
   FISDF_CHECK(c != nullptr && (on == 0 || on == 1), "set_time_reversal: on must be 0 or 1");
   c->time_reversal = on == 1;
+  return 0;
+}
+
+int fisdf_set_y_realk(fisdf_ctx* c, int on) {
+  FISDF_TRY(ctx_guard(c));
+  FISDF_CHECK(c != nullptr && on >= -1 && on <= 1, "set_y_realk: on must be -1, 0 or 1");
+  c->y_realk = on;
+  return 0;
+}
+
+int fisdf_y_real_slots(fisdf_ctx* c, int* n_real, int* n_slots) {
+  FISDF_TRY(device_guard(c));
+  FISDF_CHECK(n_real && n_slots, "y_real_slots: null argument");
+  *n_real = 0;
+  *n_slots = c->yrk_slots;
+  if (c->yrk_last < 0 || !c->yrk_dev) return 0;
+  unsigned fl[2] = {0, 0};
+  FISDF_HIP(hipMemcpyAsync(fl, c->yrk_dev + c->yrk_last * kYrkWords + 128, sizeof(fl),
+                           hipMemcpyDeviceToHost, c->stream));
+  FISDF_HIP(hipStreamSynchronize(c->stream));
+  *n_real = (int)fl[1];
   return 0;
 }
 
@@ -3834,15 +3890,18 @@
   FISDF_TRY(kmesh_check(kmesh, "y_fused_ex"));
   FISDF_TRY(check_qlist(h_qs, nq, kmesh[0] * kmesh[1] * kmesh[2], "y_fused_ex"));
   if (!y_fused_applies(kmesh, nao)) return 0;
-  const size_t yw = y_fused_workspace(kmesh, nip, nao, m);
-  FISDF_CHECK(yw > 0, "y_fused_ex: no workspace for a k-mesh the fused kernel takes");
+  const size_t yw0 = y_fused_workspace(kmesh, nip, nao, m);
+  FISDF_CHECK(yw0 > 0, "y_fused_ex: no workspace for a k-mesh the fused kernel takes");
+  const size_t yw = yw0 + y_fused_real_workspace(kmesh, nip, nao, m);
+  YfRealK rk;
+  FISDF_TRY(yrk_get(c, 0, kmesh, nao, &rk));
   char* work;
   unsigned long long* mon;
   int* dq;
   FISDF_TRY(kmesh_test_scratch(c, yw, h_qs, nq, &work, &mon, &dq));
   bool done = false;
   FISDF_TRY(y_fused(c->stream, (const cplx*)X, nip, nao, (const cplx*)F, fks, m, kmesh, h_qs, nq,
-                    (cplx*)yT, qs, Is, goff, mon, (cplx*)work, yw, rmask, &done));
+                    (cplx*)yT, qs, Is, goff, mon, (cplx*)work, yw, rmask, &done, rk));
   FISDF_HIP(hipStreamSynchronize(c->stream));
   if (h_handled) *h_handled = done ? 1 : 0;
   return 0;
@@ -3865,8 +3924,11 @@
   FISDF_TRY(kmesh_check(kmesh, "y_fused_stream_ex"));
   FISDF_TRY(check_qlist(h_qs, nq, kmesh[0] * kmesh[1] * kmesh[2], "y_fused_stream_ex"));
   if (!y_fused_applies(kmesh, nao)) return 0;
-  const size_t yw = y_fused_workspace(kmesh, nip, nao, m);
-  FISDF_CHECK(yw > 0, "y_fused_stream_ex: no workspace for a k-mesh the fused kernel takes");
+  const size_t yw0 = y_fused_workspace(kmesh, nip, nao, m);
+  FISDF_CHECK(yw0 > 0, "y_fused_stream_ex: no workspace for a k-mesh the fused kernel takes");
+  const size_t yw = yw0 + y_fused_real_workspace(kmesh, nip, nao, m);
+  YfRealK rk;
+  FISDF_TRY(yrk_get(c, 1, kmesh, nao, &rk));
   Carver cv;
   const size_t oW = cv.take(yw), oP = cv.take(sizeof(int) * ((size_t)nip + 2));
   void* base;
@@ -3892,7 +3954,7 @@
   if (rc == 0)
     rc = y_fused_stream(c->stream, (const cplx*)x0, ng0, nao, dpiv, dpiv + nip, dpiv + nip + 1, nip,
                         rows, (const cplx*)F, fks, m, kmesh, h_qs, nq, (cplx*)yT, qs, Is, goff,
-                        (cplx*)((char*)base + oW), yw, rmask, &done, s2, ea, eb);
+                        (cplx*)((char*)base + oW), yw, rmask, &done, s2, ea, eb, rk);
   int err = 0;
   if (s2) (void)hipStreamSynchronize(s2);
   if (rc == 0 && hipMemcpyAsync(&err, dpiv + nip + 1, sizeof(int), hipMemcpyDeviceToHost,
diff --git a/fft-isdf-scratch_amd/csrc/linalg.h b/fft-isdf-scratch_amd/csrc/linalg.h
--- a/fft-isdf-scratch_amd/csrc/linalg.h
+++ b/fft-isdf-scratch_amd/csrc/linalg.h
@@ -72,17 +72,22 @@
 int pair_product(hipStream_t s, const cplx* A, int n1, const cplx* B, int n2, int nip, cplx* P);
 int kmesh_half_count(const int kmesh[3]);
 size_t y_fused_workspace(const int kmesh[3], int nip, int nao, int m);
+struct YfRealK {
+  unsigned long long* stats = nullptr;
+  unsigned* flags = nullptr;
+};
+size_t y_fused_real_workspace(const int kmesh[3], int nip, int nao, int m);
 int y_fused(hipStream_t s, const cplx* X, int nip, int nao, const cplx* F, long fks, int m,
             const int kmesh[3], const int* h_qs, int nq, cplx* yT, long qs, long Is, long goff,
             unsigned long long* mon, cplx* work, size_t work_bytes, unsigned long long rmask,
-            bool* handled);
+            bool* handled, YfRealK rk = YfRealK());
 bool y_fused_applies(const int kmesh[3], int nao);
 int y_fused_stream(hipStream_t s, const cplx* x0, int ng0, int nao, const int* piv,
                    const int* progress, int* err, int nip, int rows, const cplx* F, long fks,
                    int m, const int kmesh[3], const int* h_qs, int nq, cplx* yT, long qs, long Is,
                    long goff, cplx* work, size_t work_bytes, unsigned long long rmask,
                    bool* handled, hipStream_t s2 = nullptr, hipEvent_t ev_a = nullptr,
-                   hipEvent_t ev_b = nullptr);
+                   hipEvent_t ev_b = nullptr, YfRealK rk = YfRealK());
 int kmesh_rep_runs(const int kmesh[3], std::vector<int>* runs);
 int eval_ao(hipStream_t s, const double* d_coords, int ng, int natm, const double* h_atoms, int nsh,
             const int* h_sh_atom, const int* h_sh_l, const int* h_sh_nprim, const double* h_exps,
diff --git a/fft-isdf-scratch_amd/csrc/linalg.hip b/fft-isdf-scratch_amd/csrc/linalg.hip
--- a/fft-isdf-scratch_amd/csrc/linalg.hip
+++ b/fft-isdf-scratch_amd/csrc/linalg.hip
@@ -2,6 +2,7 @@
 #include "linalg.h"
 
 #include <cmath>
+#include <type_traits>
 
 namespace fisdf {
 
@@ -493,7 +494,11 @@
   int nA, nB;
   int kA[16];
   int kB[32];
+  int nR;
+  int ordB[32];
+  int realB[32];
 };
+constexpr int YF_MAXR = 32;
 
 template <int N1, int N2>
 __host__ __device__ constexpr int yf_inplane_partner(int bc) {
@@ -506,21 +511,52 @@
   return r;
 }
 
+template <int CLS>
 __device__ __forceinline__ void yf_mfma_chunk(const cplx* __restrict__ XT, int nip, int nao,
                                               const cplx* __restrict__ FT, int m, int sbase,
-                                              int nslot, int Ia, bool okI,
-                                              int ga, bool okg, int lane, int w,
+                                              int npos, int first, const double* __restrict__ XR,
+                                              const double* __restrict__ FR, const YfPlan& plan,
+                                              unsigned passed, int Ia, bool okI,
+                                              int ga, bool okg, int lane,
                                               cplx* __restrict__ buf) {
+  constexpr bool REAL = CLS == 2;
   const int i16 = lane & 15, kq = lane >> 4;
   const int nkc = (nao + 4 * YF_MAXKS - 1) / (4 * YF_MAXKS);
-  cplx a0[YF_MAXKS], b0[YF_MAXKS], a1[YF_MAXKS], b1[YF_MAXKS];
+  typedef typename std::conditional<REAL, double, cplx>::type op_t;
+  op_t a0[YF_MAXKS], b0[YF_MAXKS], a1[YF_MAXKS], b1[YF_MAXKS];
   const int Ic = min(Ia, nip - 1), gc = min(ga, m - 1);
   (void)okI;
   (void)okg;
-  auto load = [&](cplx (&a)[YF_MAXKS], cplx (&b)[YF_MAXKS], int s, int c) {
-    const long sl = (long)(sbase + s) * nao;
-    const cplx* xa = XT + sl * nip + Ic;
-    const cplx* fb = FT + sl * m + gc;
+  auto nth_bit = [](unsigned mask, int i) {
+    for (int t = 0; t < i; ++t) mask &= mask - 1u;
+    return __builtin_ctz(mask);
+  };
+  auto place = [&](int p, int& op, int& out) {
+    if constexpr (CLS == 0) {
+      op = sbase + p;
+      out = p;
+    } else if constexpr (CLS == 2) {
+      op = nth_bit(passed, p);
+      out = plan.ordB[op];
+    } else {
+      const unsigned failed = ~passed & (plan.nR >= 32 ? ~0u : (1u << plan.nR) - 1u);
+      const int nf = __popc(failed);
+      out = plan.ordB[p < nf ? nth_bit(failed, p) : p + (plan.nR - nf)];
+      op = sbase + out;
+    }
+  };
+  auto load = [&](op_t (&a)[YF_MAXKS], op_t (&b)[YF_MAXKS], int p, int c) {
+    int op, out;
+    place(p, op, out);
+    const long sl = (long)op * nao;
+    const op_t *xa, *fb;
+    if constexpr (REAL) {
+      xa = XR + sl * nip + Ic;
+      fb = FR + sl * m + gc;
+    } else {
+      xa = XT + sl * nip + Ic;
+      fb = FT + sl * m + gc;
+    }
 #pragma unroll
     for (int kk = 0; kk < YF_MAXKS; ++kk) {
       const int mu = min(c * 4 * YF_MAXKS + kk * 4 + kq, nao - 1);
@@ -529,20 +565,27 @@
     }
   };
   f64x4 t1 = {0, 0, 0, 0}, t2 = {0, 0, 0, 0}, t3 = {0, 0, 0, 0};
-  auto mma = [&](const cplx (&a)[YF_MAXKS], const cplx (&b)[YF_MAXKS], int s, int c, int cn) {
+  auto mma = [&](const op_t (&a)[YF_MAXKS], const op_t (&b)[YF_MAXKS], int p, int c, int cn) {
 #pragma unroll
     for (int kk = 0; kk < YF_MAXKS; ++kk) {
       if (c * 4 * YF_MAXKS + kk * 4 >= nao) break;
       const bool ok = c * 4 * YF_MAXKS + kk * 4 + kq < nao;
-      const double ar = ok ? a[kk].x : 0.0, ai = ok ? a[kk].y : 0.0, br = b[kk].x, bi = b[kk].y;
-      t1 = __builtin_amdgcn_mfma_f64_16x16x4f64(ar, br, t1, 0, 0, 0);
-      t2 = __builtin_amdgcn_mfma_f64_16x16x4f64(ai, bi, t2, 0, 0, 0);
-      t3 = __builtin_amdgcn_mfma_f64_16x16x4f64(ar + ai, br - bi, t3, 0, 0, 0);
+      if constexpr (REAL) {
+        t1 = __builtin_amdgcn_mfma_f64_16x16x4f64(ok ? a[kk] : 0.0, b[kk], t1, 0, 0, 0);
+      } else {
+        const double ar = ok ? a[kk].x : 0.0, ai = ok ? a[kk].y : 0.0, br = b[kk].x, bi = b[kk].y;
+        t1 = __builtin_amdgcn_mfma_f64_16x16x4f64(ar, br, t1, 0, 0, 0);
+        t2 = __builtin_amdgcn_mfma_f64_16x16x4f64(ai, bi, t2, 0, 0, 0);
+        t3 = __builtin_amdgcn_mfma_f64_16x16x4f64(ar + ai, br - bi, t3, 0, 0, 0);
+      }
     }
     if (cn == 0) {
+      int op, out;
+      place(p, op, out);
 #pragma unroll
       for (int r = 0; r < 4; ++r)
-        buf[s * 256 + (kq + 4 * r) * 16 + i16] = cmk(t1[r] + t2[r], t3[r] - t1[r] + t2[r]);
+        buf[out * 256 + (kq + 4 * r) * 16 + i16] =
+            REAL ? cmk(t1[r], 0.0) : cmk(t1[r] + t2[r], t3[r] - t1[r] + t2[r]);
       t1 = f64x4{0, 0, 0, 0};
       t2 = f64x4{0, 0, 0, 0};
       t3 = f64x4{0, 0, 0, 0};
@@ -553,13 +596,13 @@
     cn = c + 1;
     if (cn == nkc) { sn = s + 4; cn = 0; }
   };
-  int s = __builtin_amdgcn_readfirstlane(w), c = 0, sl, cl;
-  if (s >= nslot) return;
-  auto load_item = [&](cplx (&a)[YF_MAXKS], cplx (&b)[YF_MAXKS], int si, int ci) {
-    load(a, b, min(si, nslot - 1), si < nslot ? ci : 0);
+  int s = __builtin_amdgcn_readfirstlane(first), c = 0, sl, cl;
+  if (s >= npos) return;
+  auto load_item = [&](op_t (&a)[YF_MAXKS], op_t (&b)[YF_MAXKS], int si, int ci) {
+    load(a, b, min(si, npos - 1), si < npos ? ci : 0);
   };
-  auto step = [&](cplx (&al)[YF_MAXKS], cplx (&bl)[YF_MAXKS], const cplx (&am)[YF_MAXKS],
-                  const cplx (&bm)[YF_MAXKS]) {
+  auto step = [&](op_t (&al)[YF_MAXKS], op_t (&bl)[YF_MAXKS], const op_t (&am)[YF_MAXKS],
+                  const op_t (&bm)[YF_MAXKS]) {
     load_item(al, bl, sl, cl);
     next(sl, cl, sl, cl);
     int sn, cn;
@@ -567,7 +610,7 @@
     mma(am, bm, s, c, cn);
     s = sn;
     c = cn;
-    return s < nslot;
+    return s < npos;
   };
   load(a0, b0, s, 0);
   next(s, c, sl, cl);
@@ -577,23 +620,98 @@
   }
 }
 
+__device__ __forceinline__ void yf_stats_reduce(unsigned long long mi, unsigned long long mr,
+                                                unsigned long long* __restrict__ stats) {
+  __shared__ unsigned long long red[2];
+  if (threadIdx.x < 2) red[threadIdx.x] = 0ull;
+  __syncthreads();
+#pragma unroll
+  for (int o = 32; o > 0; o >>= 1) {
+    const unsigned long long a = __shfl_xor(mi, o, 64), b = __shfl_xor(mr, o, 64);
+    mi = a > mi ? a : mi;
+    mr = b > mr ? b : mr;
+  }
+  if ((threadIdx.x & 63) == 0) {
+    if (mi) atomicMax(&red[0], mi);
+    if (mr) atomicMax(&red[1], mr);
+  }
+  __syncthreads();
+  if (threadIdx.x < 2 && red[threadIdx.x]) atomicMax(stats + threadIdx.x, red[threadIdx.x]);
+}
+__device__ __forceinline__ unsigned long long yf_absbits(double x) {
+  return (unsigned long long)__double_as_longlong(x) & 0x7fffffffffffffffull;
+}
+
 __global__ __launch_bounds__(256) void yf_transpose_kernel(const cplx* __restrict__ src,
                                                            long kstride, int nrow, int nao,
-                                                           YfPlan plan, cplx* __restrict__ dst) {
+                                                           YfPlan plan, cplx* __restrict__ dst,
+                                                           double* __restrict__ rdst,
+                                                           unsigned long long* __restrict__ stats) {
   extern __shared__ cplx tile[];
   const int j = blockIdx.y;
   const int k = j < plan.nA ? plan.kA[j] : plan.kB[j - plan.nA];
+  const int rid = (rdst && j >= plan.nA) ? plan.realB[j - plan.nA] : -1;
   const int r0 = blockIdx.x * 64, nr = min(64, nrow - r0), ld = nao + 1;
   const cplx* sp = src + (long)k * kstride + (long)r0 * nao;
+  unsigned long long mi = 0ull, mr = 0ull;
   for (int e = threadIdx.x; e < nr * nao; e += 256) {
     const int r = e / nao, mu = e - r * nao;
-    tile[r * ld + mu] = sp[e];
+    const cplx v = sp[e];
+    tile[r * ld + mu] = v;
+    const unsigned long long bi = yf_absbits(v.y), br = yf_absbits(v.x);
+    mi = bi > mi ? bi : mi;
+    mr = br > mr ? br : mr;
   }
   __syncthreads();
   cplx* dp = dst + (long)j * nao * nrow + r0;
   for (int e = threadIdx.x; e < nao * 64; e += 256) {
     const int mu = e >> 6, r = e & 63;
     if (r < nr) dp[(long)mu * nrow + r] = tile[r * ld + mu];
+  }
+  if (rid < 0) return;
+  double* rp = rdst + (long)rid * nao * nrow + r0;
+  for (int e = threadIdx.x; e < nao * 64; e += 256) {
+    const int mu = e >> 6, r = e & 63;
+    if (r < nr) rp[(long)mu * nrow + r] = tile[r * ld + mu].x;
+  }
+  if (stats) yf_stats_reduce(mi, mr, stats + 2 * rid);
+}
+
+__global__ __launch_bounds__(256) void yf_stats_kernel(const cplx* __restrict__ src, long kstride,
+                                                       long n, YfPlan plan,
+                                                       unsigned long long* __restrict__ stats) {
+  const int rid = blockIdx.y;
+  const cplx* sp = src + (long)plan.kB[plan.ordB[rid]] * kstride;
+  unsigned long long mi = 0ull, mr = 0ull;
+  for (long e = blockIdx.x * 256L + threadIdx.x; e < n; e += gridDim.x * 256L) {
+    const cplx v = sp[e];
+    const unsigned long long bi = yf_absbits(v.y), br = yf_absbits(v.x);
+    mi = bi > mi ? bi : mi;
+    mr = br > mr ? br : mr;
+  }
+  yf_stats_reduce(mi, mr, stats + 2 * rid);
+}
+
+__global__ __launch_bounds__(64) void yf_flags_kernel(unsigned long long* __restrict__ stats,
+                                                      int nR, unsigned* __restrict__ flags) {
+  const int t = threadIdx.x;
+  bool ok = false;
+  if (t < nR) {
+    ok = true;
+#pragma unroll
+    for (int op = 0; op < 2; ++op) {
+      unsigned long long* st = stats + (op * YF_MAXR + t) * 2;
+      const double im = __longlong_as_double((long long)st[0]);
+      const double re = __longlong_as_double((long long)st[1]);
+      ok = ok && im <= 64.0 * 2.220446049250313e-16 * re;
+      st[0] = 0ull;
+      st[1] = 0ull;
+    }
+  }
+  const unsigned long long b = __ballot(ok);
+  if (t == 0) {
+    flags[0] = (unsigned)b;
+    flags[1] = (unsigned)__popcll(b);
   }
 }
 
@@ -604,6 +722,7 @@
                                                            const int* __restrict__ progress,
                                                            int lo, int hi, int nip, YfPlan plan,
                                                            cplx* __restrict__ XT,
+                                                           double* __restrict__ XR,
                                                            int* __restrict__ err) {
   extern __shared__ cplx tile[];
   __shared__ int s_p[64];
@@ -639,13 +758,22 @@
     const int mu = e >> 6, r = e & 63;
     if (r < nr) dp[(long)mu * nip + r] = tile[r * ld + mu];
   }
+  const int rid = (XR && j >= plan.nA) ? plan.realB[j - plan.nA] : -1;
+  if (rid < 0) return;
+  double* rp = XR + (long)rid * nao * nip + r0;
+  for (int e = threadIdx.x; e < nao * 64; e += 256) {
+    const int mu = e >> 6, r = e & 63;
+    if (r < nr) rp[(long)mu * nip + r] = tile[r * ld + mu].x;
+  }
 }
 
 template <int N0, int N1, int N2>
 __global__ __launch_bounds__(256) __attribute__((amdgpu_waves_per_eu(2, 2))) void y_fused_kernel(
     const cplx* __restrict__ XT, int nip, int nao, const cplx* __restrict__ FT, int m,
     int nIt, int nGt, YfPlan plan, unsigned long long qmask, unsigned long long rmask,
-    cplx* __restrict__ yT, long qs, long Is, long goff, int mode, int gpair, int it0) {
+    cplx* __restrict__ yT, long qs, long Is, long goff, int mode, int gpair, int it0,
+    const double* __restrict__ XR, const double* __restrict__ FR,
+    const unsigned* __restrict__ rflag) {
   constexpr int P = N1 * N2, NK = N0 * P;
   constexpr int R = yf_inplane_rank<N1, N2>(P);
   constexpr int NC = (N0 - 1) / 2;
@@ -669,7 +797,15 @@
   for (int t = 0; t < N2; ++t) { double sn, cs; sincospi(2.0 * t / N2, &sn, &cs); tw2[t] = cmk(cs, sn); }
   cplx tc[NC > 0 ? P : 1];
   double tr[NR][P];
-  if (!(mode & 1)) yf_mfma_chunk(XT, nip, nao, FT, m, plan.nA, plan.nB, Ia, okI, ga, okg, lane, w, buf);
+  const unsigned passed = rflag ? (unsigned)__builtin_amdgcn_readfirstlane((int)*rflag) : 0u;
+  const int npass = __popc(passed);
+  if (!(mode & 1)) {
+    if (npass)
+      yf_mfma_chunk<2>(XT, nip, nao, FT, m, plan.nA, npass, w, XR, FR, plan, passed, Ia, okI, ga,
+                       okg, lane, buf);
+    yf_mfma_chunk<1>(XT, nip, nao, FT, m, plan.nA, plan.nB - npass, (w - npass) & 3, XR, FR, plan,
+                     passed, Ia, okI, ga, okg, lane, buf);
+  }
   __syncthreads();
   if (!(mode & 2)) {
 #pragma unroll
@@ -690,7 +826,9 @@
   }
   if constexpr (NC > 0) {
     __syncthreads();
-    if (!(mode & 1)) yf_mfma_chunk(XT, nip, nao, FT, m, 0, plan.nA, Ia, okI, ga, okg, lane, w, buf);
+    if (!(mode & 1))
+      yf_mfma_chunk<0>(XT, nip, nao, FT, m, 0, plan.nA, w, nullptr, nullptr, plan, 0u, Ia, okI, ga,
+                       okg, lane, buf);
     __syncthreads();
     if (mode & 2) return;
 #pragma unroll
@@ -1511,15 +1649,49 @@
       if (bc <= ((n1 - b) % n1) * n2 + (n2 - c) % n2) plan->kB[plan->nB++] = a * P + bc;
     }
   }
+  for (int i = 0; i < plan->nB; ++i) {
+    const int bc = plan->kB[i] % P, b = bc / n2, c = bc % n2;
+    const bool self = (2 * b) % n1 == 0 && (2 * c) % n2 == 0;
+    plan->realB[i] = self ? plan->nR : -1;
+    if (self) plan->ordB[plan->nR++] = i;
+  }
+  for (int i = 0, p = plan->nR; i < plan->nB; ++i)
+    if (plan->realB[i] < 0) plan->ordB[p++] = i;
   *lds = sizeof(cplx) * 256 * (size_t)std::max(plan->nA, plan->nB);
   *ok = *lds <= 80 * 1024;
+  return 0;
+}
+
+size_t y_fused_real_workspace(const int kmesh[3], int nip, int nao, int m) {
+  if (y_fused_workspace(kmesh, nip, nao, m) == 0) return 0;
+  int nR = 1;
+  for (int ax = 0; ax < 3; ++ax) nR *= kmesh[ax] % 2 == 0 ? 2 : 1;
+  return sizeof(double) * (size_t)nR * nao * ((size_t)nip + m);
+}
+
+struct YfReal {
+  double *XR = nullptr, *FR = nullptr;
+  unsigned long long* stats = nullptr;
+  unsigned* flags = nullptr;
+};
+static int yf_real_setup(const YfPlan& plan, const YfRealK& rk, cplx* work, size_t work_bytes,
+                         int nip, int nao, int m, YfReal* out) {
+  *out = YfReal{};
+  if (!rk.stats || plan.nR == 0) return 0;
+  const size_t nsl = (size_t)(plan.nA + plan.nB), base = sizeof(cplx) * nsl * nao * ((size_t)nip + m);
+  FISDF_CHECK(rk.flags && work_bytes >= base + sizeof(double) * (size_t)plan.nR * nao * ((size_t)nip + m),
+              "y_fused: workspace too small for the real slots");
+  out->XR = (double*)((char*)work + base);
+  out->FR = out->XR + (size_t)plan.nR * nao * nip;
+  out->stats = rk.stats;
+  out->flags = rk.flags;
   return 0;
 }
 
 static int yf_launch(hipStream_t s, const int kmesh[3], const cplx* XT, int nip, int nao,
                      const cplx* FT, int m, int it0, int nIt, const YfPlan& plan,
                      unsigned long long qmask, unsigned long long rmask, cplx* yT, long qs,
-                     long Is, long goff, size_t lds, bool* handled) {
+                     long Is, long goff, size_t lds, const YfReal& yr, bool* handled) {
   const int n0 = kmesh[0], n1 = kmesh[1], n2 = kmesh[2];
   const int nGt = (m + 15) / 16;
   constexpr int gpair = 4;
@@ -1532,7 +1704,7 @@
     FISDF_TRY(func_max_lds((const void*)y_fused_kernel<a, b, c>, 80 * 1024));                \
     hipLaunchKernelGGL((y_fused_kernel<a, b, c>), dim3((unsigned)grid), dim3(256), lds, s, XT,  \
                        nip, nao, FT, m, nIt, nGt, plan, qmask, rmask & qmask, yT, qs, Is, goff, \
-                       mode, gpair, it0);                                                     \
+                       mode, gpair, it0, yr.XR, yr.FR, yr.flags);                             \
     FISDF_HIP(hipGetLastError());                                                              \
     *handled = true;                                                                           \
     return 0;                                                                                  \
@@ -1545,7 +1717,7 @@
 int y_fused(hipStream_t s, const cplx* X, int nip, int nao, const cplx* F, long fks, int m,
             const int kmesh[3], const int* h_qs, int nq, cplx* yT, long qs, long Is, long goff,
             unsigned long long* mon, cplx* work, size_t work_bytes, unsigned long long rmask,
-            bool* handled) {
+            bool* handled, YfRealK rk) {
   (void)mon;
   *handled = false;
   if (m <= 0 || nip <= 0) return 0;
@@ -1560,16 +1732,22 @@
               "y_fused: workspace too small");
   cplx* XT = work;
   cplx* FT = work + (size_t)nsl * nao * nip;
+  YfReal yr;
+  FISDF_TRY(yf_real_setup(plan, rk, work, work_bytes, nip, nao, m, &yr));
   const size_t tl = sizeof(cplx) * 64 * (size_t)(nao + 1);
   FISDF_TRY(func_max_lds((const void*)yf_transpose_kernel, 132 * 1024));
   hipLaunchKernelGGL(yf_transpose_kernel, dim3((nip + 63) / 64, nsl), dim3(256), tl, s, X,
-                     (long)nip * nao, nip, nao, plan, XT);
+                     (long)nip * nao, nip, nao, plan, XT, yr.XR, yr.stats);
   FISDF_HIP(hipGetLastError());
   hipLaunchKernelGGL(yf_transpose_kernel, dim3((m + 63) / 64, nsl), dim3(256), tl, s, F, fks, m,
-                     nao, plan, FT);
-  FISDF_HIP(hipGetLastError());
+                     nao, plan, FT, yr.FR, yr.stats ? yr.stats + 2 * YF_MAXR : nullptr);
+  FISDF_HIP(hipGetLastError());
+  if (yr.stats) {
+    hipLaunchKernelGGL(yf_flags_kernel, dim3(1), dim3(64), 0, s, yr.stats, plan.nR, yr.flags);
+    FISDF_HIP(hipGetLastError());
+  }
   return yf_launch(s, kmesh, XT, nip, nao, FT, m, 0, (nip + 15) / 16, plan, qmask, rmask, yT, qs,
-                   Is, goff, lds, handled);
+                   Is, goff, lds, yr, handled);
 }
 
 bool y_fused_applies(const int kmesh[3], int nao) {
@@ -1600,7 +1778,7 @@
                    const int* progress, int* err, int nip, int rows, const cplx* F, long fks,
                    int m, const int kmesh[3], const int* h_qs, int nq, cplx* yT, long qs, long Is,
                    long goff, cplx* work, size_t work_bytes, unsigned long long rmask,
-                   bool* handled, hipStream_t s2, hipEvent_t ev_a, hipEvent_t ev_b) {
+                   bool* handled, hipStream_t s2, hipEvent_t ev_a, hipEvent_t ev_b, YfRealK rk) {
   *handled = false;
   if (m <= 0 || nip <= 0) return 0;
   FISDF_CHECK(rows >= 16 && rows % 16 == 0 && rows <= 64 * 16, "y_fused_stream: bad row block");
@@ -1617,12 +1795,22 @@
               "y_fused_stream: workspace too small");
   cplx* XT = work;
   cplx* FT = work + (size_t)nsl * nao * nip;
+  YfReal yr;
+  FISDF_TRY(yf_real_setup(plan, rk, work, work_bytes, nip, nao, m, &yr));
   const size_t tl = sizeof(cplx) * 64 * (size_t)(nao + 1);
   FISDF_TRY(func_max_lds((const void*)yf_transpose_kernel, 132 * 1024));
   FISDF_TRY(func_max_lds((const void*)yf_xt_stream_kernel, 132 * 1024));
   hipLaunchKernelGGL(yf_transpose_kernel, dim3((m + 63) / 64, nsl), dim3(256), tl, s, F, fks, m,
-                     nao, plan, FT);
-  FISDF_HIP(hipGetLastError());
+                     nao, plan, FT, yr.FR, yr.stats ? yr.stats + 2 * YF_MAXR : nullptr);
+  FISDF_HIP(hipGetLastError());
+  if (yr.stats) {
+    const long nx = (long)ng0 * nao;
+    hipLaunchKernelGGL(yf_stats_kernel, dim3((unsigned)std::min<long>((nx + 255) / 256, 256), plan.nR),
+                       dim3(256), 0, s, x0, nx, nx, plan, yr.stats);
+    FISDF_HIP(hipGetLastError());
+    hipLaunchKernelGGL(yf_flags_kernel, dim3(1), dim3(64), 0, s, yr.stats, plan.nR, yr.flags);
+    FISDF_HIP(hipGetLastError());
+  }
   if (s2) {
     FISDF_HIP(hipEventRecord(ev_a, s));
     FISDF_HIP(hipStreamWaitEvent(s2, ev_a, 0));
@@ -1631,11 +1819,11 @@
     const int hi = std::min(nip, lo + rows);
     hipStream_t sb = (s2 && (b & 1)) ? s2 : s;
     hipLaunchKernelGGL(yf_xt_stream_kernel, dim3((hi - lo + 63) / 64, nsl), dim3(256), tl, sb, x0,
-                       (long)ng0 * nao, ng0, nao, piv, progress, lo, hi, nip, plan, XT, err);
+                       (long)ng0 * nao, ng0, nao, piv, progress, lo, hi, nip, plan, XT, yr.XR, err);
     FISDF_HIP(hipGetLastError());
     bool h = false;
     FISDF_TRY(yf_launch(sb, kmesh, XT, nip, nao, FT, m, lo / 16, (hi - lo + 15) / 16, plan, qmask,
-                        rmask, yT, qs, Is, goff, lds, &h));
+                        rmask, yT, qs, Is, goff, lds, yr, &h));
     FISDF_CHECK(h, "y_fused_stream: no kernel for this k-mesh");
   }
   if (s2) {
diff --git a/fft-isdf-scratch_amd/fisdf/_lib.py b/fft-isdf-scratch_amd/fisdf/_lib.py
--- a/fft-isdf-scratch_amd/fisdf/_lib.py
+++ b/fft-isdf-scratch_amd/fisdf/_lib.py
@@ -65,6 +65,8 @@
     "fisdf_set_fit_lanes": ([_vp, _i], _i),
     "fisdf_set_factor_priority": ([_vp, _i], _i),
     "fisdf_set_time_reversal": ([_vp, _i], _i),
+    "fisdf_set_y_realk": ([_vp, _i], _i),
+    "fisdf_y_real_slots": ([_vp, _ip, _ip], _i),
     "fisdf_set_fit_pipe": ([_vp, _i, _i], _i),
     "fisdf_fit_info": ([_vp, _ip, _ip], _i),
     "fisdf_fit_report": ([_vp, _i, _ip], _i),
diff --git a/include/fisdf.h b/include/fisdf.h
--- a/include/fisdf.h
+++ b/include/fisdf.h
@@ -201,6 +201,8 @@
 int fisdf_reserve_workspace(fisdf_ctx* ctx, size_t bytes);
 int fisdf_set_omega(fisdf_ctx* ctx, double omega);
 int fisdf_set_time_reversal(fisdf_ctx* ctx, int on);
+int fisdf_set_y_realk(fisdf_ctx* ctx, int on);
+int fisdf_y_real_slots(fisdf_ctx* ctx, int* n_real, int* n_slots);
 
 int fisdf_build_ws(fisdf_ctx* ctx, const void* d_Wq, int q0, int q1, int nip,
                    const int kmesh[3], const double a[9], void* d_Ws);
```

Result: no change. 835.3, median of 6 (+0.3%).
